# MCG-NJU/SparseBEV

Hardware: AMD Instinct MI355X
Metric: decoder samples/sec (6-cam T=8 900q r50_704x256, 6 layers, features resident in HBM) (higher is better)
Workload: dtype f32 (the two mixing GEMMs: f16x3 = fp32-class (default): fp32 operands as scaled fp16 hi + lo images, 3 products (hl, lh, hh), f32 accumulate on the 16-bit matrix core (csrc/gemm_bf16s.hip); max and rms error vs fp64 below the exact f32 MFMA kernels (tests/test_gpu_bf16s.py); mixing generator + out-; 1 GPU; c2: r50_704x256, 900 queries, T=8, bs=1 per GPU, 6 decoder layers, random-init weights, NCHW (reference layout, relayout inside the step: on demand -- only the feature units the sample points read) feature input; global_batch=1, parallelism=sample-sharded x1, launches_per_layer=6, query_order=False, shuffled_queries=False, relayout=on-demand

## Files before the change

### include/sbev_hip.h

```cpp
#ifndef SBEV_HIP_H
#define SBEV_HIP_H

#include <stdint.h>

#ifdef __cplusplus
extern "C" {
#endif

#define SBEV_ABI_VERSION 1
#define SBEV_MAX_LEVELS 5
#define SBEV_MAX_POINTS 32
#define SBEV_MAX_FRAMES 16

typedef void* sbev_stream_t;

enum sbev_status {
    SBEV_OK = 0,
    SBEV_EINVAL = -1,
    SBEV_ELAUNCH = -2,
    SBEV_ENODEV = -3,
    SBEV_EFAULT = -4
};

enum sbev_dtype { SBEV_F32 = 0, SBEV_BF16 = 1, SBEV_F16 = 2, SBEV_U8 = 3 };
// ... 372 lines not shown
typedef struct sbev_decoder_config {
    int32_t B, Q, T, N, G, P, L;
    int32_t D, H, ffn;
    int32_t num_classes, code_size, num_layers, out_points;
    int32_t attn_in_rows;
    int32_t feat_dtype;
    int32_t hw[SBEV_MAX_LEVELS][2];
    float image_h, image_w, eps_homo;
    int32_t gemm_mode;
    int32_t n_slots;
    int32_t frame_slots[SBEV_MAX_FRAMES];
    int32_t overlap;
    double pc_range[6];
    const int32_t* slot_table;
} sbev_decoder_config;

typedef struct sbev_decoder_weights {
    const float *pe0_w, *pe0_b, *pe1_g, *pe1_b, *pe3_w, *pe3_b, *pe4_g, *pe4_b;
    const float *attn_in_w, *attn_in_b;
    const float *attn_out_w, *attn_out_b;
    const float *samp_w, *samp_b;
    const float *pg_w, *pg_b, *op_w, *op_b;
    const uint16_t *pg_w2, *op_w2;
    const float *ffn0_w, *ffn0_b, *ffn1_w, *ffn1_b;
    const float *norm1_g, *norm1_b, *norm2_g, *norm2_b, *norm3_g, *norm3_b;
    const float *cls0_w, *cls0_b, *cls1_g, *cls1_b, *cls3_w, *cls3_b, *cls4_g, *cls4_b, *cls6_w, *cls6_b;
    const float *reg0_w, *reg0_b, *reg2_w, *reg2_b, *reg4_w, *reg4_b;
    const float *chain_pack;
    const uint16_t *pg_ws;
    const uint16_t *op_wp;
    const float *pg_wdown;
    const float *op_nscale;
    const float *pg_xscale;
} sbev_decoder_weights;

int64_t sbev_decoder_chain_pack_floats(const sbev_decoder_config* cfg);
int sbev_decoder_chain_pack(const sbev_decoder_config* cfg, const sbev_decoder_weights* weights, float* out, sbev_stream_t stream);
int sbev_decoder_row_chain(int enable);

int sbev_decoder_chain_pair(int enable);
int64_t sbev_decoder_chain_pair_timeouts(void);
int64_t sbev_decoder_chain_pair_faults(void);
int64_t sbev_decoder_chain_pair_faults_ack(void);
int sbev_decoder_out_fold(int enable);
int sbev_linear_out8_min_rows(int rows);
int sbev_debug_out_fold_drop(int enable);
int sbev_init(void);
int sbev_debug_chain_pair_drop(int enable);

int sbev_decoder_launches_per_layer(const sbev_decoder_config* cfg, const sbev_decoder_weights* weights);

int sbev_decoder_switches(int32_t* out, int capacity);

int sbev_decoder_mixed_up_log2(const sbev_decoder_config* cfg);

int64_t sbev_decoder_workspace_bytes(const sbev_decoder_config* cfg);

int sbev_decoder_forward(const sbev_decoder_config* cfg, const sbev_decoder_weights* weights,
                         const void* const* feats_nhwc, const float* query_bbox, const float* query_feat,
                         const float* time_diff, const float* lidar2img, const float* vel_div,
                         const uint8_t* attn_mask, float* cls_out, float* bbox_out,
                         void* workspace, int64_t workspace_bytes, sbev_stream_t stream);

typedef struct sbev_lazy_feats {
    const void* const* table;
    int32_t index[SBEV_MAX_LEVELS];
    const void* src[SBEV_MAX_LEVELS];
} sbev_lazy_feats;
int sbev_decoder_lazy_supported(const sbev_decoder_config* cfg);
int sbev_decoder_lazy_scan_launch(int enable);
int sbev_decoder_forward_lazy(const sbev_decoder_config* cfg, const sbev_decoder_weights* weights, void* const* feats_nhwc,
                              const sbev_lazy_feats* lazy, const float* query_bbox, const float* query_feat,
                              const float* time_diff, const float* lidar2img, const float* vel_div,
                              const uint8_t* attn_mask, float* cls_out, float* bbox_out,
                              void* workspace, int64_t workspace_bytes, sbev_stream_t stream);
int64_t sbev_prefix_cache_bytes(const sbev_decoder_config* cfg);
int sbev_decoder_forward_cached(const sbev_decoder_config* cfg, const sbev_decoder_weights* weights, void* const* feats_nhwc,
                                const sbev_lazy_feats* lazy, const float* query_bbox, const float* query_feat,
                                const float* time_diff, const float* lidar2img, const float* vel_div,
                                const uint8_t* attn_mask, float* cls_out, float* bbox_out,
                                void* workspace, int64_t workspace_bytes, sbev_stream_t stream, void* cache, int64_t cache_bytes);
int sbev_decoder_prefix_planned(const sbev_decoder_config* cfg, const sbev_decoder_weights* weights, int cache_given, int mask_given,
                                int lazy_given);
int64_t sbev_lazy_relayout_tiles(int n_levels, const int32_t* hw_pixels, int64_t n_images, int channels);
int sbev_sample_and_project_touch(const float* query_bbox, const float* offset, int64_t ld_offset,
                                  const float* scale_logits, int64_t ld_logits,
                                  const float* time_diff, const float* lidar2img, const double* pc_range,
                                  int B, int Q, int T, int N, int G, int P, int L,
                                  float image_h, float image_w, float eps,
                                  float* loc_bp, float* weights_bp, const int32_t* hw, uint32_t* need, sbev_stream_t stream);
int sbev_nchw_to_nhwc_lazy(const void* const* table, const int32_t* index, const void* const* src, void* const* out, int n_levels,
                           const int32_t* hw_pixels, int64_t n_images, int channels, int dtype, uint32_t* need, uint32_t* done, int first,
                           int last, sbev_stream_t stream);

typedef struct sbev_graph sbev_graph;
int sbev_decoder_capture(const sbev_decoder_config* cfg, const sbev_decoder_weights* weights,
                         const void* const* feats_nhwc, const float* query_bbox, const float* query_feat,
                         const float* time_diff, const float* lidar2img, const float* vel_div,
                         const uint8_t* attn_mask, float* cls_out, float* bbox_out,
                         void* workspace, int64_t workspace_bytes, sbev_stream_t stream, sbev_graph** out);
int sbev_capture_begin(sbev_stream_t stream);
int sbev_capture_end(sbev_stream_t stream, sbev_graph** out);
int sbev_graph_launch(sbev_graph* graph, sbev_stream_t stream);
int64_t sbev_graph_num_nodes(const sbev_graph* graph);
int sbev_graph_destroy(sbev_graph* graph);

int sbev_profile_sampler(int enable);
int sbev_profile_sampler_read(float* ms, int max_n);
int sbev_profile_stride(int every_n_calls);
int sbev_profile_read(int kind, float* ms, int max_n);

enum sbev_frames_layout { SBEV_FRAMES_NCHW = 0, SBEV_FRAMES_NHWC = 1 };
int sbev_pool_insert_frames(const void* const* table, const int32_t* index, const void* const* src, void* const* out, int n_frames,
                            int n_levels, const int32_t* hw_pixels, int B, int n_views, int channels, int src_layout, int src_dtype,
                            int dst_dtype, const int32_t* insert, int n_slots, sbev_stream_t stream);

int sbev_pool_insert(const void* const* table, const int32_t* index, const void* const* src, void* const* out, int n_levels,
                     const int32_t* hw_pixels, int B, int n_views, int channels, int dtype, const int32_t* insert, int n_slots,
                     sbev_stream_t stream);

#define SBEV_FRONT_ROW_BYTES 64
int sbev_image_front_plan(int n, int H, int W, int div, int64_t* out);
int sbev_image_front(const void* src, int src_dtype, void* dst, int dst_dtype, int n, int H, int W, int div, const float* mean,
                     const float* std, int to_rgb, int colour_on, const void* table, sbev_stream_t stream);

#ifdef __cplusplus
}
#endif
#endif
```

### sparsebev_amd/_lib.py

```python
import ctypes
import os

import torch

_HERE = os.path.dirname(os.path.abspath(__file__))
LIB_PATH = os.environ.get('SBEV_LIB_PATH') or os.path.join(_HERE, 'csrc', 'libsbev_hip.so')

_c_i64p = ctypes.POINTER(ctypes.c_int64)
_c_i32p = ctypes.POINTER(ctypes.c_int32)
_vp = ctypes.c_void_p

SIGNATURES = {
    'sbev_abi_version': (ctypes.c_int, []),
    'sbev_set_box_convention': (ctypes.c_int, [ctypes.c_int]),
    'sbev_get_box_convention': (ctypes.c_int, []),
    'sbev_last_error': (ctypes.c_char_p, []),
    'sbev_device_count': (ctypes.c_int, []),
    'sbev_msmv_fwd': (ctypes.c_int, [ctypes.POINTER(_vp), _c_i32p, ctypes.c_int, ctypes.c_int,
                                     ctypes.c_int64, ctypes.c_int, ctypes.c_int, ctypes.c_int, ctypes.c_int,
                                     ctypes.c_int, _c_i64p, ctypes.c_int64, _c_i64p, ctypes.c_int64,
                                     _vp, _vp, _vp, ctypes.c_int, ctypes.c_int, ctypes.c_int, _vp]),
    'sbev_project_select': (ctypes.c_int, [_vp, _vp, ctypes.c_int, ctypes.c_int, ctypes.c_int, ctypes.c_int,
                                           ctypes.c_int, ctypes.c_int, ctypes.c_float, ctypes.c_float, ctypes.c_float,
                                           _vp, _vp, _vp, _vp, _vp]),
    'sbev_sampling_front': (ctypes.c_int, [_vp, _vp, ctypes.c_int64, _vp, ctypes.c_int64, _vp, ctypes.POINTER(ctypes.c_double),
                                           ctypes.c_int, ctypes.c_int, ctypes.c_int, ctypes.c_int, ctypes.c_int, ctypes.c_int,
                                           _vp, _vp, _vp]),
    'sbev_linear_f32': (ctypes.c_int, [_vp, _vp, _vp, _vp, _vp, ctypes.c_int64, ctypes.c_int, ctypes.c_int,
                                       ctypes.c_int64, ctypes.c_int64, ctypes.c_int64, ctypes.c_int, _vp]),
    'sbev_linear_splitk_workspace': (ctypes.c_int64, [ctypes.c_int64, ctypes.c_int, ctypes.c_int]),
    'sbev_linear_splitk_f32': (ctypes.c_int, [_vp, _vp, _vp, _vp, _vp, _vp, ctypes.c_float, _vp,
                                              ctypes.c_int64, ctypes.c_int, ctypes.c_int, ctypes.c_int64, ctypes.c_int64,
                                              ctypes.c_int, ctypes.c_int, _vp, _vp]),
    'sbev_layer_norm_f32': (ctypes.c_int, [_vp, _vp, _vp, ctypes.c_float, _vp, _vp, ctypes.c_int64, ctypes.c_int,
                                           ctypes.c_int, _vp]),
    'sbev_ln_linear_f32': (ctypes.c_int, [_vp, _vp, _vp, ctypes.c_float, ctypes.c_int, _vp, _vp, _vp, _vp, _vp, _vp,
                                          ctypes.c_int64, ctypes.c_int, ctypes.c_int, ctypes.c_int64, ctypes.c_int64,
                                          ctypes.c_int, _vp]),
    'sbev_adaptive_mixing_f32': (ctypes.c_int, [_vp, _vp, _vp, ctypes.c_int64, ctypes.c_int, ctypes.c_int, ctypes.c_int,
                                                ctypes.c_int, ctypes.c_float, _vp]),
    'sbev_sasa_f32': (ctypes.c_int, [_vp, ctypes.c_int64, _vp, ctypes.POINTER(ctypes.c_double), _vp, _vp,
                                     ctypes.c_int, ctypes.c_int, ctypes.c_int, ctypes.c_int, _vp]),
    'sbev_refine_bbox': (ctypes.c_int, [_vp, _vp, _vp, _vp, ctypes.c_int, ctypes.c_int, ctypes.c_int, _vp]),
    'sbev_nchw_to_nhwc_f32': (ctypes.c_int, [_vp, _vp, ctypes.c_int64, ctypes.c_int, ctypes.c_int, _vp]),
    'sbev_nchw_to_nhwc_f32_indirect': (ctypes.c_int, [_vp, ctypes.c_int, _vp, ctypes.c_int64, ctypes.c_int, ctypes.c_int, _vp]),
    'sbev_nchw_to_nhwc_f32_multi_indirect': (ctypes.c_int, [_vp, ctypes.c_int, _c_i32p, ctypes.POINTER(_vp), ctypes.c_int64, ctypes.c_int, _c_i32p, _vp]),
    'sbev_nchw_to_nhwc_b16': (ctypes.c_int, [_vp, _vp, ctypes.c_int64, ctypes.c_int, ctypes.c_int, _vp]),
    'sbev_nchw_to_nhwc_b16_indirect': (ctypes.c_int, [_vp, ctypes.c_int, _vp, ctypes.c_int64, ctypes.c_int, ctypes.c_int, _vp]),
    'sbev_copy_indirect': (ctypes.c_int, [_vp, ctypes.c_int, _c_i32p, ctypes.POINTER(_vp), _c_i64p, _vp]),
    'sbev_finish_outputs': (ctypes.c_int, [_vp, _vp, _vp, _vp, ctypes.c_int64, ctypes.c_int64, _vp]),
    'sbev_finish_outputs_indirect': (ctypes.c_int, [_vp, ctypes.c_int, ctypes.c_int, _vp, _vp, ctypes.c_int64, ctypes.c_int64, _vp]),
    'sbev_linear3_ln_relu_f32': (ctypes.c_int, [_vp, ctypes.c_int64, _vp, _vp, _vp, _vp, ctypes.c_float, _vp,
                                                ctypes.c_int64, ctypes.c_int, _vp]),
    'sbev_decoder_workspace_bytes': (ctypes.c_int64, [_vp]),
    'sbev_decoder_launches_per_layer': (ctypes.c_int, [_vp, _vp]),
    'sbev_decoder_switches': (ctypes.c_int, [_c_i32p, ctypes.c_int]),
    'sbev_decoder_forward': (ctypes.c_int, [_vp, _vp, ctypes.POINTER(_vp), _vp, _vp, _vp, _vp, _vp, _vp, _vp, _vp,
                                            _vp, ctypes.c_int64, _vp]),
    'sbev_decoder_forward_lazy': (ctypes.c_int, [_vp, _vp, ctypes.POINTER(_vp), _vp, _vp, _vp, _vp, _vp, _vp, _vp, _vp, _vp,
                                                 _vp, ctypes.c_int64, _vp]),
    'sbev_decoder_forward_cached': (ctypes.c_int, [_vp, _vp, ctypes.POINTER(_vp), _vp, _vp, _vp, _vp, _vp, _vp, _vp, _vp, _vp,
                                                   _vp, ctypes.c_int64, _vp, _vp, ctypes.c_int64]),
    'sbev_prefix_cache_bytes': (ctypes.c_int64, [_vp]),
    'sbev_decoder_prefix_planned': (ctypes.c_int, [_vp, _vp, ctypes.c_int, ctypes.c_int, ctypes.c_int]),
    'sbev_decoder_lazy_supported': (ctypes.c_int, [_vp]),
    'sbev_decoder_lazy_scan_launch': (ctypes.c_int, [ctypes.c_int]),
    'sbev_lazy_relayout_tiles': (ctypes.c_int64, [ctypes.c_int, _c_i32p, ctypes.c_int64, ctypes.c_int]),
    'sbev_sample_and_project_touch': (ctypes.c_int, [_vp, _vp, ctypes.c_int64, _vp, ctypes.c_int64, _vp, _vp,
                                                     ctypes.POINTER(ctypes.c_double), ctypes.c_int, ctypes.c_int, ctypes.c_int,
                                                     ctypes.c_int, ctypes.c_int, ctypes.c_int, ctypes.c_int,
                                                     ctypes.c_float, ctypes.c_float, ctypes.c_float, _vp, _vp, _c_i32p, _vp, _vp]),
    'sbev_nchw_to_nhwc_lazy': (ctypes.c_int, [_vp, _c_i32p, ctypes.POINTER(_vp), ctypes.POINTER(_vp), ctypes.c_int, _c_i32p, ctypes.c_int64,
                                              ctypes.c_int, ctypes.c_int, _vp, _vp, ctypes.c_int, ctypes.c_int, _vp]),
    'sbev_init': (ctypes.c_int, []),
    'sbev_decoder_out_fold': (ctypes.c_int, [ctypes.c_int]),
    'sbev_linear_out8_min_rows': (ctypes.c_int, [ctypes.c_int]),
    'sbev_debug_out_fold_drop': (ctypes.c_int, [ctypes.c_int]),
    'sbev_profile_sampler': (ctypes.c_int, [ctypes.c_int]),
    'sbev_profile_stride': (ctypes.c_int, [ctypes.c_int]),
    'sbev_profile_sampler_read': (ctypes.c_int, [ctypes.POINTER(ctypes.c_float), ctypes.c_int]),
    'sbev_splitk_reduce_f32': (ctypes.c_int, [_vp, ctypes.c_int, _vp, _vp, _vp, _vp, ctypes.c_float, _vp, ctypes.c_int64,
                                              ctypes.c_int, ctypes.c_int, _vp]),
    'sbev_split_bf16x3_weights': (ctypes.c_int, [_vp, _vp, ctypes.c_int64, ctypes.c_int, _vp]),
    'sbev_linear_bf16x3_strip_ok': (ctypes.c_int, [ctypes.c_int64, ctypes.c_int, ctypes.c_int]),
    'sbev_linear_bf16x3_strip': (ctypes.c_int, [_vp, _vp, _vp, _vp, ctypes.c_int64, ctypes.c_int, ctypes.c_int, ctypes.c_int64,
                                                ctypes.c_int, _vp]),
    'sbev_linear_bf16x3': (ctypes.c_int, [_vp, _vp, _vp, _vp, _vp, ctypes.c_int64, ctypes.c_int, ctypes.c_int,
                                          ctypes.c_int64, ctypes.c_int64, ctypes.c_int, _vp]),
    'sbev_linear_splitk_bf16x3': (ctypes.c_int, [_vp, _vp, _vp, _vp, _vp, _vp, ctypes.c_float, _vp, ctypes.c_int64, ctypes.c_int,
                                                 ctypes.c_int, ctypes.c_int64, ctypes.c_int, ctypes.c_int, _vp, _vp]),
    'sbev_bf16s_image_elems': (ctypes.c_int64, [ctypes.c_int64, ctypes.c_int, ctypes.c_int]),
    'sbev_split_bf16s_rows': (ctypes.c_int, [_vp, ctypes.c_int64, _vp, ctypes.c_int64, ctypes.c_int, ctypes.c_int, _vp]),
    'sbev_pack_bf16s_frags': (ctypes.c_int, [_vp, ctypes.c_int64, _vp, ctypes.c_int, ctypes.c_int, ctypes.c_int, _vp]),
    'sbev_linear_gen_weight_stationary': (ctypes.c_int, [ctypes.c_int]),
    'sbev_linear_bf16s_gen_ok': (ctypes.c_int, [ctypes.c_int64, ctypes.c_int, ctypes.c_int]),
    'sbev_linear_bf16s_gen': (ctypes.c_int, [_vp, _vp, _vp, _vp, ctypes.c_int64, ctypes.c_int, ctypes.c_int, ctypes.c_int64,
                                             ctypes.c_int, ctypes.c_int, _vp]),
    'sbev_decoder_mixed_up_log2': (ctypes.c_int, [_vp]),
    'sbev_pack_f16s_frags': (ctypes.c_int, [_vp, ctypes.c_int64, _vp, _vp, ctypes.c_int, ctypes.c_int, ctypes.c_int, _vp]),
    'sbev_linear_f16s_gen': (ctypes.c_int, [_vp, _vp, _vp, _vp, _vp, _vp, ctypes.c_int64, ctypes.c_int, ctypes.c_int, ctypes.c_int64,
                                            ctypes.c_int, ctypes.c_int, _vp]),
    'sbev_f16s_pairs': (ctypes.c_int, [_vp, _vp, ctypes.c_int64, ctypes.c_int, _vp]),
    'sbev_f16s_tensor_scale': (ctypes.c_int, [_vp, ctypes.c_int64, ctypes.c_int64, ctypes.c_int, _vp, _vp]),
    'sbev_gemm_tn_f16s_ok': (ctypes.c_int, [ctypes.c_int64, ctypes.c_int64, ctypes.c_int64]),
    'sbev_gemm_tn_f16s': (ctypes.c_int, [_vp, ctypes.c_int64, _vp, _vp, ctypes.c_int64, _vp, _vp, ctypes.c_int64,
                                         ctypes.c_int64, ctypes.c_int64, ctypes.c_int64, ctypes.c_int, _vp]),
    'sbev_adaptive_mixing_bwd_max_f32': (ctypes.c_int, [_vp, _vp, _vp, _vp, _vp, _vp, ctypes.c_int64, ctypes.c_int, ctypes.c_int, ctypes.c_int,
                                                        ctypes.c_int, ctypes.c_float, _vp]),
    'sbev_adaptive_mixing_pairs_f16': (ctypes.c_int, [_vp, _vp, _vp, ctypes.c_int64, ctypes.c_int, ctypes.c_int, ctypes.c_int, ctypes.c_int,
                                                      ctypes.c_float, ctypes.c_int, _vp]),
    'sbev_linear_splitk_f16s': (ctypes.c_int, [_vp, ctypes.c_int, ctypes.c_int, _vp, _vp, _vp, _vp, _vp, _vp, ctypes.c_float, _vp, ctypes.c_int64, ctypes.c_int,
                                               ctypes.c_int, ctypes.c_int64, ctypes.c_int, ctypes.c_int, _vp, _vp]),
    'sbev_f16s_out_scale': (ctypes.c_int, [_vp, ctypes.c_int, _vp, ctypes.c_int, _vp]),
    'sbev_linear_splitk_f16s_xdev': (ctypes.c_int, [_vp, _vp, _vp, _vp, _vp, _vp, _vp, _vp, ctypes.c_float, _vp, ctypes.c_int64, ctypes.c_int,
                                                    ctypes.c_int, ctypes.c_int64, ctypes.c_int, ctypes.c_int, _vp, _vp]),
    'sbev_linear_bf16s_out_ok': (ctypes.c_int, [ctypes.c_int64, ctypes.c_int, ctypes.c_int]),
    'sbev_linear_bf16s_out_plan': (ctypes.c_int, [ctypes.c_int64, ctypes.c_int, ctypes.c_int]),
    'sbev_linear_gen_plan': (ctypes.c_int, [ctypes.c_int64, ctypes.c_int, ctypes.c_int, ctypes.c_int64, ctypes.c_int, ctypes.c_int, ctypes.c_int,
                                            _c_i32p, ctypes.c_int]),
    'sbev_linear_splitk_bf16s': (ctypes.c_int, [_vp, _vp, _vp, _vp, _vp, _vp, ctypes.c_float, _vp, ctypes.c_int64, ctypes.c_int,
                                                ctypes.c_int, ctypes.c_int64, ctypes.c_int, ctypes.c_int, _vp, _vp]),
    'sbev_msmv_bwd': (ctypes.c_int, [ctypes.POINTER(_vp), ctypes.POINTER(_vp), _c_i32p, ctypes.c_int,
                                     ctypes.c_int64, ctypes.c_int, ctypes.c_int, ctypes.c_int, ctypes.c_int,
                                     ctypes.c_int, _c_i64p, ctypes.c_int64, _c_i64p, ctypes.c_int64,
                                     _vp, _vp, _vp, _vp, _vp, _vp]),
    'sbev_msmv_fwd_ring': (ctypes.c_int, [ctypes.POINTER(_vp), _c_i32p, ctypes.c_int, ctypes.c_int,
                                          ctypes.c_int64, ctypes.c_int, ctypes.c_int, ctypes.c_int, ctypes.c_int,
                                          ctypes.c_int, _c_i64p, ctypes.c_int64, _c_i64p, ctypes.c_int64,
                                          _vp, _vp, _vp, ctypes.c_int, ctypes.c_int, ctypes.c_int, _c_i32p, ctypes.c_int, _vp]),
    'sbev_msmv_fwd_pool': (ctypes.c_int, [ctypes.POINTER(_vp), _c_i32p, ctypes.c_int, ctypes.c_int,
                                          ctypes.c_int64, ctypes.c_int, ctypes.c_int, ctypes.c_int, ctypes.c_int,
                                          ctypes.c_int, _c_i64p, ctypes.c_int64, _c_i64p, ctypes.c_int64,
                                          _vp, _vp, _vp, ctypes.c_int, ctypes.c_int, ctypes.c_int, _vp, ctypes.c_int, _vp]),
    'sbev_sample_mix_pool': (ctypes.c_int, [ctypes.POINTER(_vp), _c_i32p, ctypes.c_int, ctypes.c_int,
                                            ctypes.c_int64, ctypes.c_int, ctypes.c_int, ctypes.c_int, ctypes.c_int, ctypes.c_int, ctypes.c_int,
                                            _c_i64p, ctypes.c_int64, _c_i64p, ctypes.c_int64, _vp, _vp, _c_i32p, _vp, ctypes.c_int,
                                            _vp, _vp, ctypes.c_int, ctypes.c_float, ctypes.c_int, ctypes.c_int, _vp, _vp]),
    'sbev_sample_and_project': (ctypes.c_int, [_vp, _vp, ctypes.c_int64, _vp, ctypes.c_int64, _vp, _vp,
                                               ctypes.POINTER(ctypes.c_double), ctypes.c_int, ctypes.c_int, ctypes.c_int,
                                               ctypes.c_int, ctypes.c_int, ctypes.c_int, ctypes.c_int,
                                               ctypes.c_float, ctypes.c_float, ctypes.c_float, _vp, _vp, _vp]),
    'sbev_decoder_capture': (ctypes.c_int, [_vp, _vp, ctypes.POINTER(_vp), _vp, _vp, _vp, _vp, _vp, _vp, _vp, _vp, _vp, ctypes.c_int64, _vp, _vp]),
    'sbev_capture_begin': (ctypes.c_int, [_vp]),
    'sbev_capture_end': (ctypes.c_int, [_vp, _vp]),
    'sbev_graph_launch': (ctypes.c_int, [_vp, _vp]),
    'sbev_graph_num_nodes': (ctypes.c_int64, [_vp]),
    'sbev_graph_destroy': (ctypes.c_int, [_vp]),
# ... 167 lines not shown
```

### sparsebev_amd/csrc/decoder.hip

```cpp
#include <atomic>
#include <cmath>
#include <cstdlib>
#include <cstring>
#include "sbev_common.hpp"

#include <mutex>
#include <vector>

namespace {

struct Carver {
    char* base;
    size_t off = 0;
    explicit Carver(void* p) : base(static_cast<char*>(p)) {}
    float* take(size_t n_floats) {
        float* r = reinterpret_cast<float*>(base + off);
        off += (n_floats * sizeof(float) + 255) / 256 * 256;
        return r;
    }
};

struct Buffers {
    float *t0, *t1, *x, *x1, *x2, *x3, *qkvt, *att, *so, *wbp, *loc, *sampled, *params, *mixed, *slabs,
        *h, *c0, *c1, *r0, *r1, *reg, *bbox, *x1s, *xsc, *pair_x, *folded;
    uint32_t* pair_sync;
    int32_t* order;
    uint32_t *touch_need, *touch_done;
    size_t bytes;
};

bool lazy_plan_of(const sbev_decoder_config& c, sbev::LazyPlan* p) {
    if (c.n_slots > 0 || c.G != 4 || c.D != 256) return false;
    int32_t s[SBEV_MAX_LEVELS];
    for (int l = 0; l < c.L; ++l) s[l] = c.hw[l][0] * c.hw[l][1];
    return sbev::lazy_plan(c.L, s, (long long)c.B * c.T * c.N, c.D, p);
}

int out_proj_splits(long long M, int N, int K) { return sbev_linear_splitk_plan(M, N, K); }

Buffers carve(const sbev_decoder_config& c, void* ws) {
    Carver k(ws);
    const size_t BQ = (size_t)c.B * c.Q, D = c.D;
    const int Cg = c.D / c.G, Pin = c.T * c.P;
    const size_t pgN = (size_t)c.G * (Cg * Cg + Pin * c.out_points);
    const size_t mixN = (size_t)c.G * c.out_points * Cg;
    Buffers b{};
    b.t0 = k.take(BQ * D); b.t1 = k.take(BQ * D);
    b.x = k.take(BQ * D); b.x1 = k.take(BQ * D); b.x2 = k.take(BQ * D); b.x3 = k.take(BQ * D);
    b.qkvt = k.take(BQ * (size_t)c.attn_in_rows);
    b.att = k.take(BQ * D);
    b.so = k.take(BQ * (size_t)(c.G * c.P * (3 + c.L)));
    b.wbp = k.take(BQ * c.T * c.G * c.P * c.L);
    b.loc = k.take(BQ * c.T * c.G * c.P * 3);
    b.sampled = k.take(BQ * c.G * Pin * Cg);
    b.params = k.take(BQ * pgN);
    b.mixed = k.take(BQ * mixN);
    {
        int sl = out_proj_splits(BQ, c.D, (int)mixN);
        const int sl2 = sbev_linear_bf16s_out_plan((int64_t)BQ, c.D, (int)mixN);
        sl = sl2 > sl ? sl2 : sl;
        b.slabs = k.take((size_t)sl * BQ * D);
    }
    b.h = k.take(BQ * c.ffn);
    b.c0 = k.take(BQ * D); b.c1 = k.take(BQ * D); b.r0 = k.take(BQ * D); b.r1 = k.take(BQ * D);
    b.reg = k.take(BQ * c.code_size);
    b.bbox = k.take(BQ * 10);
    b.x1s = k.take(2 * BQ * D + 64 * (size_t)D);
    b.xsc = k.take(64);
    b.pair_x = k.take((size_t)sbev::chain_pair_floats((long long)BQ));
    b.pair_sync = reinterpret_cast<uint32_t*>(k.take((size_t)sbev::chain_pair_sync_words((long long)BQ)));
    b.order = reinterpret_cast<int32_t*>(k.take(BQ));
    b.folded = k.take(BQ * D);
    sbev::LazyPlan lp;
    if (lazy_plan_of(c, &lp)) {
        b.touch_need = reinterpret_cast<uint32_t*>(k.take(lp.base[lp.n_levels]));
        b.touch_done = reinterpret_cast<uint32_t*>(k.take(lp.base[lp.n_levels]));
    }
    b.bytes = k.off;
    return b;
}

struct Prefix {
    uint32_t* hdr;
    float *qb, *qf, *x0, *att0, *params0;
    size_t bytes;
};
Prefix carve_prefix(const sbev_decoder_config& c, void* cache) {
    Carver k(cache);
    const size_t BQ = (size_t)c.B * c.Q, D = c.D;
    const int Cg = c.D / c.G, Pin = c.T * c.P;
    Prefix f{};
    f.hdr = reinterpret_cast<uint32_t*>(k.take(sbev::PFX_DIRTY + sbev::PFX_NW));
    f.qb = k.take(BQ * 10);
    f.qf = k.take(BQ * D);
    f.x0 = k.take(BQ * D);
    f.att0 = k.take(BQ * D);
    f.params0 = k.take(BQ * (size_t)c.G * (Cg * Cg + Pin * c.out_points));
    f.bytes = k.off;
    return f;
}

struct WatchArgs {
    const uint32_t* q[2];
    uint32_t* copy[2];
    uint32_t words[2];
    uint32_t* hdr;
};
__global__ __launch_bounds__(256) void prefix_watch_kernel(const WatchArgs a) {
    const uint32_t armed = a.hdr[sbev::PFX_ARMED], force = a.hdr[sbev::PFX_FORCE];
    uint32_t differed = 0;
#pragma unroll
    for (int s = 0; s < 2; ++s) {
        const uint4* q = reinterpret_cast<const uint4*>(a.q[s]);
        uint4* cp = reinterpret_cast<uint4*>(a.copy[s]);
        const uint32_t n16 = a.words[s] / 4;
        for (uint32_t i = blockIdx.x * 256u + threadIdx.x; i < n16; i += sbev::PFX_NW * 256u) {
            const uint4 v = q[i], o = cp[i];
            if (((v.x ^ o.x) | (v.y ^ o.y)) | ((v.z ^ o.z) | (v.w ^ o.w))) {
                cp[i] = v;
                differed = 1;
            }
        }
        const uint32_t t = 4 * n16 + threadIdx.x;
        if (blockIdx.x == 0 && t < a.words[s] && a.q[s][t] != a.copy[s][t]) {
            a.copy[s][t] = a.q[s][t];
            differed = 1;
        }
    }
    const int any = __syncthreads_or((int)differed);
    if (threadIdx.x == 0) {
        a.hdr[sbev::PFX_DIRTY + blockIdx.x] = (any != 0 || armed == 0 || force != 0) ? 1u : 0u;
        if (blockIdx.x == 0) a.hdr[sbev::PFX_ARMED] = 1u;
    }
}

std::atomic<int> g_fuse_sample_mix{1};
std::atomic<int> g_fuse_l5_f32{getenv("SBEV_NO_FUSE_L5F32") ? 0 : 1};

std::atomic<int> g_query_order{getenv("SBEV_QUERY_ORDER") ? (atoi(getenv("SBEV_QUERY_ORDER")) == 2 ? 2 : atoi(getenv("SBEV_QUERY_ORDER")) != 0) : 0};

std::atomic<int> g_row_chain{1};
std::atomic<int> g_lazy_scan_launch{getenv("SBEV_LAZY_SCAN_LAUNCH") ? 1 : 0};

int validate(const sbev_decoder_config* c) {
    SBEV_REQUIRE(c != nullptr, "sbev_decoder: null config");
    SBEV_REQUIRE(c->B >= 1 && c->Q >= 1 && c->T >= 1 && c->N >= 1 && c->G >= 1 && c->P >= 1, "sbev_decoder: bad sizes");
    SBEV_REQUIRE(c->L >= 1 && c->L <= SBEV_MAX_LEVELS, "sbev_decoder: num_levels %d", c->L);
    SBEV_REQUIRE(c->D % (4 * c->G) == 0 && c->D % c->H == 0 && c->D / c->H == 32, "sbev_decoder: embed_dims %d / heads %d (head_dim must be 32)", c->D, c->H);
    SBEV_REQUIRE(c->D / c->G == 64 && c->out_points == 128, "sbev_decoder: built for 64 channels per group and 128 out points");
    SBEV_REQUIRE(c->attn_in_rows >= 3 * c->D + c->H && c->attn_in_rows % 4 == 0, "sbev_decoder: attn_in_rows %d", c->attn_in_rows);
    SBEV_REQUIRE(c->code_size == 10, "sbev_decoder: code_size %d (the box kernels are built for the 10-wide box code)", c->code_size);
    SBEV_REQUIRE(c->num_layers >= 1 && c->num_classes >= 1 && c->ffn % 4 == 0, "sbev_decoder: head sizes");
    SBEV_REQUIRE(c->gemm_mode >= SBEV_GEMM_F32 && c->gemm_mode <= SBEV_GEMM_F16X4, "sbev_decoder: gemm_mode %d", c->gemm_mode);
    SBEV_REQUIRE(!c->slot_table || (c->n_slots > 0 && c->T <= SBEV_MAX_FRAMES), "sbev_decoder: slot_table (keyed frame pool) needs n_slots > 0 and T <= %d",
                 SBEV_MAX_FRAMES);
    return SBEV_OK;
}

struct Aux {
    hipStream_t stream = nullptr;
    hipEvent_t ev[8] = {};
    bool ok = false;
};
Aux& aux() {
    static Aux a;
    static std::once_flag once;
    std::call_once(once, [] {
        bool ok = hipStreamCreateWithFlags(&a.stream, hipStreamNonBlocking) == hipSuccess;
        for (auto& e : a.ev) ok = ok && hipEventCreateWithFlags(&e, hipEventDisableTiming) == hipSuccess;
        a.ok = ok;
    });
    return a;
}
inline int hip_ok(hipError_t e, const char* what) {
    if (e == hipSuccess) return SBEV_OK;
    sbev::set_error("%s: %s", what, hipGetErrorString(e));
    return SBEV_ELAUNCH;
}

struct ConfigPyramid {
    int64_t sbo[SBEV_MAX_LEVELS], sv[SBEV_MAX_LEVELS];
    sbev::PyramidDesc d;
    ConfigPyramid(const sbev_decoder_config& c, const void* const* feats, const float* loc, const float* weights)
        : d{feats, &c.hw[0][0], c.L, c.feat_dtype, c.N, c.D / c.G, c.Q, c.P, c.G, sbo, c.D / c.G, sv, c.D, loc, weights,
            c.n_slots > 0 && !c.slot_table ? c.frame_slots : nullptr, c.n_slots, c.slot_table} {
        for (int l = 0; l < c.L; ++l) {
            sv[l] = (int64_t)c.hw[l][0] * c.hw[l][1] * c.D;
            sbo[l] = sv[l] * c.N;
        }
    }
    ConfigPyramid(const ConfigPyramid&) = delete;
};

#define TRY(expr)                 \
    do {                          \
        int st__ = (expr);        \
        if (st__ != SBEV_OK) return st__; \
    } while (0)

}

static bool launch_profiling_on();

namespace sbev {
struct ProfCallScope {
    bool prev;
    ProfCallScope();
    ~ProfCallScope();
};
// ... 22 lines not shown
    return s;
}

extern "C" int sbev_decoder_switches(int32_t* out, int capacity) {
    constexpr int n = (int)(sizeof(sbev::Switches) / sizeof(int32_t));
    static_assert(sizeof(sbev::Switches) == n * sizeof(int32_t), "sbev::Switches: int32_t fields only");
    const sbev::Switches s = read_switches();
    if (out && capacity > 0) std::memcpy(out, &s, sizeof(int32_t) * (capacity < n ? capacity : n));
    return n;
}

struct StepPlan {
    int nimg;
    int64_t BQ;
    int pgN, mixN, soN;
    int splits;
    bool fork, fork_pg;
    bool chain;
    bool fused;
    int order_mode;
    bool pg_strip;
    bool pack_launch;
    bool gen_ws;
    bool scan_in_gen;
    bool fold_wanted;
    bool grouped;
    bool prefix;
    int out8_min_rows;
    int launches_per_layer;
};

static StepPlan plan_step(const sbev_decoder_config& c, const sbev_decoder_weights& w, bool lazy, bool aux_ok, const sbev::Switches& sw,
                          bool cache_usable = false) {
    StepPlan p{};
    p.nimg = c.gemm_mode == SBEV_GEMM_BF16X6 ? 3 : c.gemm_mode == SBEV_GEMM_BF16X3S ? 2 : c.gemm_mode == SBEV_GEMM_F16X3 ? 4
             : c.gemm_mode == SBEV_GEMM_F16X4 ? 5 : 0;
    const int D = c.D, Cg = c.D / c.G, Pin = c.T * c.P;
    p.BQ = (int64_t)c.B * c.Q;
    p.pgN = c.G * (Cg * Cg + Pin * c.out_points);
    p.mixN = c.G * c.out_points * Cg;
    p.soN = c.G * c.P * (3 + c.L);
    p.splits = out_proj_splits(p.BQ, D, p.mixN);
    p.fork = c.overlap != 0 && aux_ok;
    p.fork_pg = c.overlap == 1 && aux_ok;
    p.chain = sw.row_chain != 0 && w.chain_pack != nullptr && !p.fork && sbev::row_chain_supported(c) && sbev::row_chain_pays(p.BQ);
    p.fused = sw.fuse_sample_mix != 0 && sample_mix_fusable(c, sw.fuse_l5_f32 != 0);
    p.order_mode = p.chain && p.fused && c.Q <= sbev_query_order_max() ? sw.query_order : 0;
    p.pg_strip = c.gemm_mode == SBEV_GEMM_BF16X3 && sbev_linear_bf16x3_strip_ok(p.BQ, p.pgN, D) != 0;
    p.pack_launch = p.nimg ? !(p.nimg >= 4 && p.chain) : p.pg_strip;
    p.gen_ws = p.nimg != 0 && sw.gen_weight_stationary != 0 && sbev::gen_ws_shape_ok(p.BQ, D, p.pgN, p.nimg);
    p.scan_in_gen = lazy && p.chain && p.nimg >= 4 && sw.lazy_scan_launch == 0 && p.BQ <= 1024 && p.gen_ws;
    p.fold_wanted = p.chain && p.nimg >= 4 && sw.chain_pair != 0 && sw.out_fold != 0;
    p.grouped = !p.fork && (D == 256 || D == 512) && ((p.BQ + 127) / 128) * ((D + 127) / 128) < 256;
    p.out8_min_rows = sw.out8_min_rows;
    p.prefix = cache_usable && p.chain && p.gen_ws;
    p.launches_per_layer = (p.chain ? 6 : 17) + (p.fused ? 0 : 1) + (p.pack_launch ? 1 : 0) + (p.order_mode == 1 ? 1 : 0);
    return p;
}

extern "C" int sbev_decoder_launches_per_layer(const sbev_decoder_config* cfg, const sbev_decoder_weights* w) {
    if (validate(cfg) != SBEV_OK || !w) return -1;
    return plan_step(*cfg, *w, false, true, read_switches()).launches_per_layer;
}

extern "C" int sbev_decoder_mixed_up_log2(const sbev_decoder_config* cfg) {
    if (!cfg || cfg->G < 1 || cfg->out_points < 1 || cfg->D < cfg->G) return 0;
    const double bound = std::sqrt((double)cfg->out_points * (cfg->D / cfg->G));
    int e = 0;
    while (std::ldexp(bound, e + 1) < 65504.0 && e < 15) ++e;
    return e;
}

extern "C" int64_t sbev_prefix_cache_bytes(const sbev_decoder_config* cfg) {
    if (validate(cfg) != SBEV_OK) return -1;
    return (int64_t)carve_prefix(*cfg, nullptr).bytes;
}

extern "C" int sbev_decoder_prefix_planned(const sbev_decoder_config* cfg, const sbev_decoder_weights* w, int cache_given, int mask_given,
                                           int lazy_given) {
    if (validate(cfg) != SBEV_OK || !w) return -1;
    return plan_step(*cfg, *w, lazy_given != 0, true, read_switches(), cache_given && !mask_given && !launch_profiling_on()).prefix ? 1 : 0;
}

extern "C" int64_t sbev_decoder_workspace_bytes(const sbev_decoder_config* cfg) {
    if (validate(cfg) != SBEV_OK) return -1;
    sbev::chain_pair_prepare();
    return (int64_t)carve(*cfg, nullptr).bytes;
}

namespace {

struct Step {
    const sbev_decoder_config& c;
    const sbev_decoder_weights& w;
    const StepPlan& p;
    const Buffers& b;
    const void* const* feats_nhwc;
    const float *query_bbox, *query_feat, *time_diff, *lidar2img, *vel_div;
    const uint8_t* attn_mask;
    float *cls_out, *bbox_out;
    const sbev_lazy_feats* lazy;
    const Prefix* pf;
    sbev_stream_t stream;
    Aux& ax;
    hipStream_t s_main = reinterpret_cast<hipStream_t>(stream);
    sbev_stream_t s_aux = p.fork ? reinterpret_cast<sbev_stream_t>(ax.stream) : stream;
    int evi = 0;
    sbev::LazyPlan lplan{};
    const ConfigPyramid pyramid{c, feats_nhwc, b.loc, b.wbp};
    const int mixed_up = sbev_decoder_mixed_up_log2(&c), D = c.D, Cg = c.D / c.G, Pin = c.T * c.P;
    const float eps = 1e-5f;
    const float* bbox = query_bbox;
    const float* feat = query_feat;
    bool pe0_done = false;
    hipEvent_t ev_cls = nullptr;
    float* params = b.params;
    const uint32_t* skip = nullptr;

    float* cls_of(int layer) const { return cls_out + (int64_t)layer * p.BQ * c.num_classes; }
    float* box_of(int layer) const { return bbox_out + (int64_t)layer * p.BQ * c.code_size; }
    int feat_esize() const { return c.feat_dtype == SBEV_F32 ? 4 : 2; }

    int fork_to_aux() {
        hipEvent_t e = ax.ev[(evi++) & 7];
        TRY(hip_ok(hipEventRecord(e, s_main), "hipEventRecord"));
        return hip_ok(hipStreamWaitEvent(ax.stream, e, 0), "hipStreamWaitEvent");
    }
    int record_on_aux(hipEvent_t* ev) {
        *ev = ax.ev[(evi++) & 7];
        return hip_ok(hipEventRecord(*ev, ax.stream), "hipEventRecord");
    }
    int join(hipEvent_t ev) { return ev ? hip_ok(hipStreamWaitEvent(s_main, ev, 0), "hipStreamWaitEvent") : SBEV_OK; }
    sbev::LazyScan lazy_scan(int layer) const {
        if (!lazy) return {};
        return {&lplan, lazy->table, lazy->index, lazy->src, const_cast<void* const*>(feats_nhwc), feat_esize(), b.touch_need, b.touch_done,
                layer + 1 == c.num_layers};
    }
    int lazy_move(const sbev::LazyScan& scan, bool first) { return scan.plan ? sbev::launch_lazy_relayout(scan, first, s_main) : SBEV_OK; }

    int generator_bf16x3(sbev_stream_t st) {
        if (!p.pg_strip) return sbev_linear_bf16x3(b.x1, w.pg_w2, w.pg_b, nullptr, params, p.BQ, p.pgN, D, D, p.pgN, 0, st);
        uint16_t* x2 = reinterpret_cast<uint16_t*>(b.x1s);
        TRY(sbev_split_bf16x3_weights(b.x1, x2, p.BQ, D, st));
        return sbev_linear_bf16x3_strip(x2, w.pg_w2, w.pg_b, params, p.BQ, p.pgN, D, p.pgN, 0, st);
    }
    int generator_bf16s(sbev_stream_t st, const sbev::LazyScan* scan) {
        uint16_t* xs = reinterpret_cast<uint16_t*>(b.x1s);
        if (p.pack_launch) {
            TRY(p.nimg >= 4 ? sbev_pack_f16s_frags(b.x1, D, xs, const_cast<float*>(w.pg_xscale), (int)p.BQ, D, 2, st)
                            : sbev_pack_bf16s_frags(b.x1, D, xs, (int)p.BQ, D, p.nimg, st));
        }
        return sbev::launch_gen_gemm({{xs, w.pg_xscale}, {w.pg_ws, w.pg_wdown}, w.pg_b, params, p.BQ, p.pgN, D, p.pgN, 0, p.nimg, p.gen_ws, scan, skip},
                                     reinterpret_cast<hipStream_t>(st));
    }
    int generator(sbev_stream_t st, const sbev::LazyScan* scan) {
        if (p.nimg) return generator_bf16s(st, scan);
        if (c.gemm_mode == SBEV_GEMM_BF16X3) return generator_bf16x3(st);
        return sbev_linear_f32(b.x1, w.pg_w, w.pg_b, nullptr, params, p.BQ, p.pgN, D, D, D, p.pgN, 0, st);
    }

    int gather(sbev_stream_t st) {
        return sbev::msmv_fwd(pyramid.d, (int64_t)c.B * c.T * c.G, b.sampled, SBEV_OUT_MIX, c.T, c.G, st);
    }
    int gather_and_mix(sbev_stream_t st, const int32_t* order, hipEvent_t params_ready = nullptr) {
        if (!p.fused) TRY(gather(st));
        TRY(join(params_ready));
        if (!p.fused && p.nimg >= 4) return sbev_adaptive_mixing_pairs_f16(b.sampled, params, b.mixed, p.BQ, c.G, Pin, Cg, c.out_points, eps, mixed_up, st);
        if (!p.fused) return sbev_adaptive_mixing_f32(b.sampled, params, b.mixed, p.BQ, c.G, Pin, Cg, c.out_points, eps, st);
        return sbev::sample_mix(pyramid.d, c.B, c.T, c.G, params, b.mixed, c.out_points, eps, p.nimg >= 4 ? ldexpf(1.f, mixed_up) : 0.f, order, st);
    }

    int out_projection_slabs(sbev::OutProjResult* r) {
        *r = {0, false};
        if (p.nimg) {
            const bool f16 = p.nimg >= 4;
            const bool fold = p.fold_wanted && sbev::out_fold_shape_ok(p.BQ, p.mixN) && sbev::chain_fault_word_ready();
            const sbev::OutProj o{{f16 ? sbev::SplitImageX::F16_PAIRS : sbev::SplitImageX::F32_HOST_EXP, b.mixed, p.mixN, f16 ? mixed_up : 0, nullptr},
                                  w.op_wp, f16 ? w.op_nscale : nullptr, p.BQ, p.mixN, p.nimg, b.slabs, p.out8_min_rows,
                                  fold ? b.pair_sync + sbev::chain_fold_sync_offset(p.BQ) : nullptr, fold ? b.folded : nullptr};
            return sbev::launch_out_proj_slabs(o, r, s_main);
        }
        if (c.gemm_mode == SBEV_GEMM_BF16X3)
            return sbev::launch_splitk_slabs_bf16x3(b.mixed, w.op_w2, p.BQ, D, p.mixN, p.mixN, p.splits, b.slabs, &r->used, s_main);
        return sbev::launch_splitk_slabs(b.mixed, w.op_w, p.BQ, D, p.mixN, p.mixN, p.mixN, p.splits, b.slabs, &r->used, s_main);
    }
    int out_projection(sbev_stream_t st) {
        if (p.nimg >= 4)
            return sbev_linear_splitk_f16s(b.mixed, 1, mixed_up, w.op_wp, w.op_nscale, w.op_b, b.x1, w.norm2_g, w.norm2_b, eps, b.x2, p.BQ, D, p.mixN,
                                           p.mixN, 0, p.nimg - 1, b.slabs, st);
        if (p.nimg)
            return sbev_linear_splitk_bf16s(b.mixed, w.op_wp, w.op_b, b.x1, w.norm2_g, w.norm2_b, eps, b.x2, p.BQ, D, p.mixN, p.mixN,
                                            0, p.nimg, b.slabs, st);
        if (c.gemm_mode == SBEV_GEMM_BF16X3)
            return sbev_linear_splitk_bf16x3(b.mixed, w.op_w2, w.op_b, b.x1, w.norm2_g, w.norm2_b, eps, b.x2, p.BQ, D, p.mixN, p.mixN,
                                             0, p.splits, b.slabs, st);
        return sbev_linear_splitk_f32(b.mixed, w.op_w, w.op_b, b.x1, w.norm2_g, w.norm2_b, eps, b.x2, p.BQ, D, p.mixN, p.mixN, p.mixN,
                                      0, p.splits, b.slabs, st);
    }

    int layer_chain(int layer) {
        if (p.order_mode != 0 && (layer == 0 || p.order_mode == 1)) TRY(sbev_query_order(bbox, c.code_size, c.pc_range, c.B, c.Q, b.order, stream));
        const bool cached = pf && layer == 0;
        float* att = cached ? pf->att0 : b.att;
        params = cached ? pf->params0 : b.params;
        skip = cached ? pf->hdr : nullptr;
        TRY(sbev::launch_sasa(b.qkvt, c.attn_in_rows, bbox, c.pc_range, attn_mask, att, c.B, c.Q, c.H, D / c.H, skip, s_main));
        TRY(sbev::launch_chain_attn(c, w, att, cached ? pf->x0 : b.x, b.x1, bbox, time_diff, lidar2img, b.loc, b.wbp, eps, s_main,
                                    p.nimg >= 4 ? reinterpret_cast<uint16_t*>(b.x1s) : nullptr, p.nimg >= 4 ? w.pg_xscale : nullptr, b.pair_sync,
                                    lazy ? &lplan : nullptr, lazy ? b.touch_need : nullptr));
        const bool ride = p.scan_in_gen && layer > 0;
        SBEV_REQUIRE(!(ride && skip), "sbev_decoder_forward: a generator that carries a relayout scan cannot skip");
        const sbev::LazyScan scan = lazy_scan(layer);
        if (!ride) TRY(lazy_move(scan, layer == 0));
        TRY(generator(stream, ride ? &scan : nullptr));
        TRY(gather_and_mix(stream, p.order_mode != 0 ? b.order : nullptr));
        sbev::OutProjResult op;
        TRY(out_projection_slabs(&op));
        TRY(sbev::launch_chain_tail(c, w, op.folded ? b.folded : b.slabs, op.used, b.x1, bbox, c.T > 1 ? vel_div : nullptr, b.x3, cls_of(layer), box_of(layer),
                                    layer + 1 < c.num_layers, b.x, b.qkvt, eps, s_main, b.pair_x, b.pair_sync));
        bbox = box_of(layer);
        return SBEV_OK;
    }

    int layer_ops(int layer) {
        if (!pe0_done) TRY(sbev_linear3_ln_relu_f32(bbox, layer == 0 ? 10 : c.code_size, w.pe0_w, w.pe0_b, w.pe1_g, w.pe1_b, eps, b.t0, p.BQ, D, stream));
        pe0_done = false;
        TRY(sbev_linear_f32(b.t0, w.pe3_w, w.pe3_b, nullptr, b.t1, p.BQ, D, D, D, D, D, 0, stream));
        TRY(sbev_ln_linear_f32(b.t1, w.pe4_g, w.pe4_b, eps, 1, feat, b.x, w.attn_in_w, w.attn_in_b, nullptr, b.qkvt,
                               p.BQ, c.attn_in_rows, D, D, c.attn_in_rows, 0, stream));
        TRY(sbev_sasa_f32(b.qkvt, c.attn_in_rows, bbox, c.pc_range, attn_mask, b.att, c.B, c.Q, c.H, D / c.H, stream));
        TRY(sbev_linear_f32(b.att, w.attn_out_w, w.attn_out_b, b.x, b.t1, p.BQ, D, D, D, D, D, 0, stream));
        TRY(sbev_ln_linear_f32(b.t1, w.norm1_g, w.norm1_b, eps, 0, nullptr, b.x1, w.samp_w, w.samp_b, nullptr, b.so,
                               p.BQ, p.soN, D, D, p.soN, 0, stream));
        hipEvent_t ev_pg = nullptr;
        if (p.fork_pg) TRY(fork_to_aux());
        TRY(generator(p.fork_pg ? s_aux : stream, nullptr));
        if (p.fork_pg) TRY(record_on_aux(&ev_pg));
        TRY(sbev::launch_sample_and_project(bbox, b.so, p.soN, b.so + c.G * c.P * 3, p.soN, time_diff, lidar2img, c.pc_range,
                                            c.B, c.Q, c.T, c.N, c.G, c.P, c.L, c.image_h, c.image_w, c.eps_homo, b.loc, b.wbp,
                                            lazy ? &lplan : nullptr, lazy ? b.touch_need : nullptr, c.hw, s_main));
        TRY(lazy_move(lazy_scan(layer), layer == 0));
        TRY(gather_and_mix(stream, nullptr, ev_pg));
        TRY(out_projection(stream));
        TRY(join(ev_cls));
        TRY(sbev_linear_f32(b.x2, w.ffn0_w, w.ffn0_b, nullptr, b.h, p.BQ, c.ffn, D, D, D, c.ffn, 1, stream));
        TRY(sbev_linear_f32(b.h, w.ffn1_w, w.ffn1_b, b.x2, b.t1, p.BQ, D, c.ffn, c.ffn, c.ffn, D, 0, stream));
        TRY(p.grouped ? branches_grouped(layer) : branches_forked(layer));
        bbox = box_of(layer);
        feat = b.x3;
        return SBEV_OK;
    }

    sbev_linear_problem problem(const float* X, const float* W, const float* bias, float* Y, int N, int relu) const {
        return sbev_linear_problem{X, W, bias, nullptr, Y, p.BQ, N, D, D, D, N, relu};
    }
    int branches_grouped(int layer) {
        const bool ln_fused = sbev::ln_linear_fusable(p.BQ, D, D);
        if (!ln_fused) TRY(sbev_layer_norm_f32(b.t1, w.norm3_g, w.norm3_b, eps, nullptr, b.x3, p.BQ, D, 0, stream));
        const float* x = ln_fused ? b.t1 : b.x3;
        const sbev_linear_problem g1[2] = {problem(x, w.cls0_w, w.cls0_b, b.c0, D, 0), problem(x, w.reg0_w, w.reg0_b, b.r0, D, 1)};
        const sbev::LnPrologue norm3{w.norm3_g, w.norm3_b, eps, 0, nullptr, b.x3};
        TRY(ln_fused ? sbev::launch_linear_group(g1, 2, &norm3, s_main) : sbev_linear_group_f32(g1, 2, stream));
        TRY(sbev::launch_ln_and_linear(b.c0, w.cls1_g, w.cls1_b, eps, 1, b.c1, p.BQ, D, b.r0, w.reg2_w, w.reg2_b, b.r1, D, D, 1, s_main));
        const sbev_linear_problem g2[2] = {problem(b.c1, w.cls3_w, w.cls3_b, b.c0, D, 0), problem(b.r1, w.reg4_w, w.reg4_b, b.reg, c.code_size, 0)};
        TRY(sbev_linear_group_f32(g2, 2, stream));
        TRY(sbev::launch_ln_and_refine(b.c0, w.cls4_g, w.cls4_b, eps, 1, b.c1, p.BQ, D,
                                       bbox, b.reg, c.T > 1 ? vel_div : nullptr, box_of(layer), c.Q, c.code_size, s_main));
        if (layer + 1 == c.num_layers)
            return sbev_linear_f32(b.c1, w.cls6_w, w.cls6_b, nullptr, cls_of(layer), p.BQ, c.num_classes, D, D, D, c.num_classes, 0, stream);
        TRY(sbev::launch_linear_and_lin3(b.c1, w.cls6_w, w.cls6_b, cls_of(layer), p.BQ, c.num_classes, D, 0,
                                         box_of(layer), c.code_size, w.pe0_w, w.pe0_b, w.pe1_g, w.pe1_b, eps, b.t0, D, s_main));
        pe0_done = true;
        return SBEV_OK;
    }
    int branches_forked(int layer) {
        TRY(sbev_ln_linear_f32(b.t1, w.norm3_g, w.norm3_b, eps, 0, nullptr, b.x3, w.cls0_w, w.cls0_b, nullptr, b.c0,
                               p.BQ, D, D, D, D, 0, stream));
        if (p.fork) TRY(fork_to_aux());
        TRY(sbev_layer_norm_f32(b.c0, w.cls1_g, w.cls1_b, eps, nullptr, b.c1, p.BQ, D, 1, s_aux));
        TRY(sbev_linear_f32(b.c1, w.cls3_w, w.cls3_b, nullptr, b.c0, p.BQ, D, D, D, D, D, 0, s_aux));
        TRY(sbev_layer_norm_f32(b.c0, w.cls4_g, w.cls4_b, eps, nullptr, b.c1, p.BQ, D, 1, s_aux));
        TRY(sbev_linear_f32(b.c1, w.cls6_w, w.cls6_b, nullptr, cls_of(layer), p.BQ, c.num_classes, D, D, D, c.num_classes, 0, s_aux));
        if (p.fork) TRY(record_on_aux(&ev_cls));
        TRY(sbev_linear_f32(b.x3, w.reg0_w, w.reg0_b, nullptr, b.r0, p.BQ, D, D, D, D, D, 1, stream));
        TRY(sbev_linear_f32(b.r0, w.reg2_w, w.reg2_b, nullptr, b.r1, p.BQ, D, D, D, D, D, 1, stream));
        TRY(sbev_linear_f32(b.r1, w.reg4_w, w.reg4_b, nullptr, b.reg, p.BQ, c.code_size, D, D, D, c.code_size, 0, stream));
        return sbev_refine_bbox(bbox, b.reg, c.T > 1 ? vel_div : nullptr, box_of(layer), c.B, c.Q, c.code_size, stream);
    }

    int prefix_watch() {
        const WatchArgs a{{reinterpret_cast<const uint32_t*>(query_bbox), reinterpret_cast<const uint32_t*>(query_feat)},
                          {reinterpret_cast<uint32_t*>(pf->qb), reinterpret_cast<uint32_t*>(pf->qf)},
                          {(uint32_t)(p.BQ * 10), (uint32_t)(p.BQ * D)}, pf->hdr};
        hipLaunchKernelGGL(prefix_watch_kernel, dim3(sbev::PFX_NW), dim3(256), 0, s_main, a);
        return sbev::check_launch("prefix cache (watch)");
    }

    int run() {
        if (pf) TRY(prefix_watch());
        if (p.chain) TRY(sbev::launch_chain_front(c, w, query_bbox, query_feat, pf ? pf->x0 : b.x, b.qkvt, eps, s_main, pf ? pf->hdr : nullptr));
        for (int layer = 0; layer < c.num_layers; ++layer) TRY(p.chain ? layer_chain(layer) : layer_ops(layer));
        return join(ev_cls);
    }
};

}

static int decoder_forward_impl(const sbev_decoder_config* cfg, const sbev_decoder_weights* w,
                                const void* const* feats_nhwc, const float* query_bbox, const float* query_feat,
                                const float* time_diff, const float* lidar2img, const float* vel_div,
                                const uint8_t* attn_mask, float* cls_out, float* bbox_out,
                                void* workspace, int64_t workspace_bytes, sbev_stream_t stream, const sbev_lazy_feats* lazy,
                                void* cache = nullptr, int64_t cache_bytes = 0) {
    TRY(validate(cfg));
    const sbev_decoder_config& c = *cfg;
    SBEV_REQUIRE(w && feats_nhwc && query_bbox && query_feat && time_diff && lidar2img && cls_out && bbox_out && workspace,
                 "sbev_decoder_forward: null pointer");
    if (const unsigned faults = sbev::chain_pair_faults_pending()) {
        sbev_decoder_chain_pair(0);
        sbev::set_error("sbev_decoder_forward: %u pair-mode hand-off(s) of an EARLIER decoder step timed out -- that step's outputs are invalid; "
                        "pair mode is now off: acknowledge with sbev_decoder_chain_pair_faults_ack() and repeat the step", faults);
        return SBEV_EFAULT;
    }
    const sbev::ProfCallScope prof_scope;
    Aux& ax = aux();
    const bool cache_usable = cache && !attn_mask && !launch_profiling_on() && ((((uintptr_t)query_bbox) | ((uintptr_t)query_feat)) & 15) == 0;
    const StepPlan p = plan_step(c, *w, lazy != nullptr, ax.ok, read_switches(), cache_usable);
    SBEV_REQUIRE((((uintptr_t)workspace) & 255) == 0, "sbev_decoder_forward: workspace must be 256-byte aligned");
    SBEV_REQUIRE(cfg->gemm_mode != SBEV_GEMM_BF16X3 || (w->pg_w2 && w->op_w2), "sbev_decoder_forward: gemm_mode bf16x3 needs pg_w2 / op_w2");
    SBEV_REQUIRE(p.nimg == 0 || (w->pg_ws && w->op_wp), "sbev_decoder_forward: gemm_mode %d needs pg_ws / op_wp", cfg->gemm_mode);
    SBEV_REQUIRE(p.nimg < 4 || (w->pg_wdown && w->op_nscale && w->pg_xscale), "sbev_decoder_forward: gemm_mode %d needs pg_wdown / op_nscale / pg_xscale", cfg->gemm_mode);
    const Buffers b = carve(c, workspace);
    SBEV_REQUIRE((int64_t)b.bytes <= workspace_bytes, "sbev_decoder_forward: workspace too small (%lld < %zu)", (long long)workspace_bytes, b.bytes);

    Prefix pf{};
    if (p.prefix) {
        pf = carve_prefix(c, cache);
        SBEV_REQUIRE((((uintptr_t)cache) & 255) == 0, "sbev_decoder_forward_cached: cache must be 256-byte aligned");
        SBEV_REQUIRE((int64_t)pf.bytes <= cache_bytes, "sbev_decoder_forward_cached: cache too small (%lld < %zu)", (long long)cache_bytes, pf.bytes);
        SBEV_REQUIRE(p.BQ * (int64_t)c.D < 0x7fffffffLL, "sbev_decoder_forward_cached: too many query words");
    }
    Step step{c, *w, p, b, feats_nhwc, query_bbox, query_feat, time_diff, lidar2img, vel_div, attn_mask, cls_out, bbox_out, lazy,
              p.prefix ? &pf : nullptr, stream, ax};
    if (lazy) {
        SBEV_REQUIRE(lazy_plan_of(c, &step.lplan) && b.touch_need, "sbev_decoder_forward_lazy: config not covered (dense pyramid, 4 groups of 64 channels)");
        for (int l = 0; l < c.L; ++l)
            SBEV_REQUIRE(feats_nhwc[l] && (((uintptr_t)feats_nhwc[l]) & 15) == 0 &&
                         (lazy->table ? lazy->index[l] >= 0 : (lazy->src[l] && (((uintptr_t)lazy->src[l]) & 15) == 0 && lazy->src[l] != feats_nhwc[l])),
                         "sbev_decoder_forward_lazy: level %d (16-byte aligned NCHW source and NHWC destination)", l);
        SBEV_REQUIRE(!lazy->table || (((uintptr_t)lazy->table) & 7) == 0, "sbev_decoder_forward_lazy: unaligned pointer table");
    }
    SBEV_REQUIRE(p.nimg == 0 || (sbev_linear_bf16s_gen_ok(p.BQ, p.pgN, c.D) && sbev_linear_bf16s_out_ok(p.BQ, c.D, p.mixN)),
                 "sbev_decoder_forward: gemm_mode %d does not cover this shape (rows %lld, generator %d x %d, out-projection %d x %d)",
                 cfg->gemm_mode, (long long)p.BQ, p.pgN, c.D, c.D, p.mixN);
    return step.run();
}

extern "C" int sbev_decoder_forward(const sbev_decoder_config* cfg, const sbev_decoder_weights* w,
                                    const void* const* feats_nhwc, const float* query_bbox, const float* query_feat,
                                    const float* time_diff, const float* lidar2img, const float* vel_div,
                                    const uint8_t* attn_mask, float* cls_out, float* bbox_out,
                                    void* workspace, int64_t workspace_bytes, sbev_stream_t stream) {
    return decoder_forward_impl(cfg, w, feats_nhwc, query_bbox, query_feat, time_diff, lidar2img, vel_div, attn_mask, cls_out, bbox_out, workspace,
                                workspace_bytes, stream, nullptr);
}

extern "C" int sbev_decoder_forward_lazy(const sbev_decoder_config* cfg, const sbev_decoder_weights* w, void* const* feats_nhwc,
                                         const sbev_lazy_feats* lazy, const float* query_bbox, const float* query_feat,
                                         const float* time_diff, const float* lidar2img, const float* vel_div,
                                         const uint8_t* attn_mask, float* cls_out, float* bbox_out,
                                         void* workspace, int64_t workspace_bytes, sbev_stream_t stream) {
    SBEV_REQUIRE(lazy, "sbev_decoder_forward_lazy: null source descriptor");
    return decoder_forward_impl(cfg, w, const_cast<const void* const*>(feats_nhwc), query_bbox, query_feat, time_diff, lidar2img, vel_div, attn_mask,
                                cls_out, bbox_out, workspace, workspace_bytes, stream, lazy);
}

extern "C" int sbev_decoder_forward_cached(const sbev_decoder_config* cfg, const sbev_decoder_weights* w, void* const* feats_nhwc,
                                           const sbev_lazy_feats* lazy, const float* query_bbox, const float* query_feat,
                                           const float* time_diff, const float* lidar2img, const float* vel_div,
                                           const uint8_t* attn_mask, float* cls_out, float* bbox_out,
                                           void* workspace, int64_t workspace_bytes, sbev_stream_t stream, void* cache, int64_t cache_bytes) {
    return decoder_forward_impl(cfg, w, const_cast<const void* const*>(feats_nhwc), query_bbox, query_feat, time_diff, lidar2img, vel_div, attn_mask,
                                cls_out, bbox_out, workspace, workspace_bytes, stream, lazy, cache, cache_bytes);
}

extern "C" int sbev_decoder_lazy_supported(const sbev_decoder_config* cfg) {
    sbev::LazyPlan p;
    return cfg && validate(cfg) == SBEV_OK && lazy_plan_of(*cfg, &p) ? 1 : 0;
}

namespace sbev {
static std::mutex g_prof_mu;
static int g_prof_mask = 0;
static int g_prof_stride = 1;
static long long g_prof_calls = 0;
static thread_local bool tl_prof_skip = false;
struct ProfEvent { hipEvent_t e0, e1; int kind; };
static std::vector<ProfEvent> g_prof_events;

bool profile_begin(hipStream_t s, hipEvent_t* e0, hipEvent_t* e1, int kind) {
    std::lock_guard<std::mutex> lk(g_prof_mu);
    if (!((g_prof_mask >> kind) & 1) || tl_prof_skip) return false;
    if (hipEventCreate(e0) != hipSuccess || hipEventCreate(e1) != hipSuccess) return false;
    (void)hipEventRecord(*e0, s);
    return true;
}
void profile_end(hipStream_t s, hipEvent_t e0, hipEvent_t e1, int kind) {
    (void)hipEventRecord(e1, s);
    std::lock_guard<std::mutex> lk(g_prof_mu);
    g_prof_events.push_back({e0, e1, kind});
}
}

static bool launch_profiling_on() {
    std::lock_guard<std::mutex> lk(sbev::g_prof_mu);
    return sbev::g_prof_mask != 0;
}

namespace sbev {
ProfCallScope::ProfCallScope() : prev(tl_prof_skip) {
    std::lock_guard<std::mutex> lk(g_prof_mu);
    if (g_prof_mask != 0 && g_prof_stride > 1) tl_prof_skip = (g_prof_calls++ % g_prof_stride) != 0;
}
ProfCallScope::~ProfCallScope() { tl_prof_skip = prev; }
}

extern "C" int sbev_profile_stride(int every_n_calls) {
    SBEV_REQUIRE(every_n_calls >= 1, "sbev_profile_stride: need n >= 1 (got %d)", every_n_calls);
    std::lock_guard<std::mutex> lk(sbev::g_prof_mu);
    sbev::g_prof_stride = every_n_calls;
    sbev::g_prof_calls = 0;
    return SBEV_OK;
}

extern "C" int sbev_decoder_lazy_scan_launch(int enable) { return g_lazy_scan_launch.exchange(enable ? 1 : 0, std::memory_order_relaxed); }

extern "C" int sbev_decoder_row_chain(int enable) {
    g_row_chain.store(enable != 0, std::memory_order_relaxed);
    return SBEV_OK;
}

extern "C" int sbev_decoder_fuse_sample_mix(int enable) {
    g_fuse_sample_mix.store(enable ? 1 : 0, std::memory_order_relaxed);
    return SBEV_OK;
}

extern "C" int sbev_decoder_query_order(int enable) {
    return g_query_order.exchange(enable == 2 ? 2 : enable ? 1 : 0, std::memory_order_relaxed);
}

extern "C" int sbev_profile_sampler(int enable) {
    std::lock_guard<std::mutex> lk(sbev::g_prof_mu);
    sbev::g_prof_mask = enable;
    return SBEV_OK;
}

extern "C" int sbev_profile_read(int kind, float* ms, int max_n) {
    std::lock_guard<std::mutex> lk(sbev::g_prof_mu);
    int n = 0;
    std::vector<sbev::ProfEvent> keep;
    for (auto& ev : sbev::g_prof_events) {
        if (ev.kind != kind) {
            keep.push_back(ev);
            continue;
        }
        float t = 0.f;
// ... 106 lines not shown
```

### sparsebev_amd/csrc/row_chain.hip

```cpp
#include "sbev_common.hpp"
#include "sample_point.hpp"
#include <mutex>
#include <atomic>
#include <cstdlib>

namespace {

constexpr int NWAVE = 8;
constexpr int DM = 256, FF = 512;
constexpr int LDX = DM + 8;
constexpr int LDH = FF + 8;
static_assert(2 * LDX >= LDH, "branch rows alias the ffn hidden rows");

constexpr int PV_OP_B = 0, PV_N2G = 256, PV_N2B = 512, PV_FFN0_B = 768, PV_FFN1_B = 1280, PV_N3G = 1536, PV_N3B = 1792,
              PV_CLS0_B = 2048, PV_CLS1G = 2304, PV_CLS1B = 2560, PV_CLS3_B = 2816, PV_CLS4G = 3072, PV_CLS4B = 3328,
              PV_CLS6_B = 3584, PV_REG0_B = 3648, PV_REG2_B = 3904, PV_REG4_B = 4160, PV_TAIL_END = 4224;
constexpr int PV_PE0_W = PV_TAIL_END, PV_PE0_B = PV_PE0_W + 768, PV_PE1G = PV_PE0_B + 256, PV_PE1B = PV_PE1G + 256,
              PV_PE3_B = PV_PE1B + 256, PV_PE4G = PV_PE3_B + 256, PV_PE4B = PV_PE4G + 256, PV_QKV_B = PV_PE4B + 256, PV_QKV_PAD = 832,
              PV_FRONT_END = PV_QKV_B + PV_QKV_PAD;
constexpr int PV_AOUT_B = 0, PV_N1G = 256, PV_N1B = 512, PV_SAMP_B = 768, PV_ATTN_END = 1024;
constexpr int PV_IMAGE_FLOATS = PV_FRONT_END + PV_ATTN_END;

enum Epi { EPI_FFN0, EPI_FFN1, EPI_BR1, EPI_BR2, EPI_OUT, EPI_PE3, EPI_QKV, EPI_AOUT, EPI_SAMP };
enum Pre { PRE_SLABS, PRE_FRONT, PRE_ATT };

struct Lin {
    const float* wp;
    int in_off, ld;
    int KH;
    int items;
    int chunks;
    int kh0, KHT;
};
struct Unit {
    Lin a, b;
    int epi;
    int col0;
};

#ifdef SBEV_CHAIN_TRACE
#define SBEV_TRACE(i) if ((blockIdx.x == 7 || blockIdx.x == 15) && lane == 0) a.trace[(blockIdx.x == 15 ? 64 * 512 : 0) + wave * 64 + (i)] = (long long)__builtin_amdgcn_s_memrealtime();
#else
#define SBEV_TRACE(i)
#endif

struct ChainArgs {
#ifdef SBEV_CHAIN_TRACE
    long long* trace;
#endif
    Unit units[8];
    Unit units_b[8];
    int n_units, pre, front;
    int n_pairs;
    float* pair_x;
    unsigned* pair_sync;
    unsigned* zero_words; int n_zero;
    int debug_drop;
    const float* warm;
    int warm_lines;
    const float* vec;
    int vec_off, vec_n;
    long long M;
    int Q;
    const float* slabs; int splits;
    const float* x1;
    float* x3;
    const float* bbox;
    const float* vel_div;
    float* cls_out;
    float* box_out;
    int num_classes;
    const float* feat;
    float* x;
    float* qkvt; int attn_in_rows;
    const float* att;
    float* x1_out;
    unsigned short* x1_frag;
    const float* x1_scale;
    float* so; int soN;
    sbev_ops::SamplePointArgs proj;
    float eps;
    uint32_t* skip_hdr;
};

constexpr int RING_SLOTS = 3;
constexpr int CHUNK_FLOATS = 1024;

template <int RG>
struct Lay {
    static constexpr int R = 4 * RG;
    static constexpr bool WIDE = RG > 1;
    static constexpr int MAX_SLOTS = WIDE ? 12 : 16;
    static constexpr int OFF_X2 = 0;
    static constexpr int OFF_X3 = OFF_X2 + R * LDX;
    static constexpr int OFF_H = OFF_X3 + R * LDX;
    static constexpr int OFF_C = OFF_H;
    static constexpr int OFF_R = OFF_H + R * LDX;
    static constexpr int OFF_P = OFF_H + 2 * R * LDX;
    static constexpr int LDS_FLOATS = OFF_P + MAX_SLOTS * R * 64;
    static constexpr int OFF_RING = LDS_FLOATS;
    static constexpr int OFF_DUMP = OFF_RING + (WIDE ? 0 : NWAVE * RING_SLOTS * CHUNK_FLOATS);
    static constexpr int OFF_PARAM = OFF_DUMP + NWAVE * 64;
    static constexpr int LDS_TOTAL_FLOATS = OFF_PARAM + PV_FRONT_END;
    static constexpr int RPW = (R + NWAVE - 1) / NWAVE;
    static_assert(LDS_TOTAL_FLOATS * 4 <= 160 * 1024, "LDS budget of one CU");
};
struct Offs { int x2, x3, h, c, r; };
template <int RG> constexpr Offs offs_of() { return Offs{Lay<RG>::OFF_X2, Lay<RG>::OFF_X3, Lay<RG>::OFF_H, Lay<RG>::OFF_C, Lay<RG>::OFF_R}; }

template <int RG>
__device__ __forceinline__ void warm_l2(const ChainArgs& a, int wave, int lane) {
    const int per_xcd = ((int)gridDim.x + 7) / 8;
    const int parts = per_xcd < 32 ? per_xcd : 32;
    const int part = ((int)blockIdx.x / 8) % parts;
    const int n = (a.warm_lines + parts - 1) / parts;
    const int l0 = part * n;
    const int l1 = min(a.warm_lines, l0 + n);
    const unsigned dump = (unsigned)(Lay<RG>::OFF_DUMP + wave * 64) * 4u;
    for (int l = l0 + wave * 64; l < l1; l += NWAVE * 64) {
        const int line = min(l + lane, l1 - 1);
        const unsigned voff = (unsigned)line * 128u;
        asm volatile(
            "s_mov_b32 m0, %0\n\t"
            "s_nop 0\n\t"
            "global_load_lds_dword %1, %2\n\t"
            :
            : "s"(dump), "v"(voff), "s"(a.warm)
            : "memory");
    }
}

struct Walk {
    int u, it, step;
};

__device__ __forceinline__ int unit_items(const Unit* U, int u) { return U[u].a.items + U[u].b.items; }

__device__ __forceinline__ void walk_settle(const ChainArgs& a, const Unit* U, Walk& w, int wave) {
    while (w.u < a.n_units && w.it >= unit_items(U, w.u)) {
        ++w.u;
        w.it = wave;
    }
}

__device__ __forceinline__ const float* item_weights(const Unit& un, int it) {
    const bool second = it >= un.a.items;
    const Lin& l = second ? un.b : un.a;
    const int j = it - (second ? un.a.items : 0);
    const int piece = l.KHT == l.KH ? j : (j / l.KH) * l.KHT + l.kh0 + j % l.KH;
    return l.wp + (long long)piece * (l.chunks * CHUNK_FLOATS);
}

__device__ __forceinline__ void issue_chunk(const float* g, unsigned lds_byte, unsigned voff) {
    asm volatile(
        "s_mov_b32 m0, %0\n\t"
        "s_nop 0\n\t"
        "global_load_lds_dwordx4 %1, %2\n\t"
        "global_load_lds_dwordx4 %1, %2 offset:1024\n\t"
        "global_load_lds_dwordx4 %1, %2 offset:2048\n\t"
        "global_load_lds_dwordx4 %1, %2 offset:3072\n\t"
        :
        : "s"(lds_byte), "v"(voff), "s"(g)
        : "memory");
}

struct Stream {
// ... 146 lines not shown
#pragma unroll
        for (int kh = 0; kh < KH; ++kh) t[c][kh] = P[(base + (cg0 + c) * KH + kh) * (R * 64) + row * 64 + lane];
#pragma unroll
    for (int c = 0; c < 4; ++c) {
        float s = 0.f;
#pragma unroll
        for (int kh = 0; kh < KH; ++kh) s += t[c][kh];
        v[c] = s + bias[bias0 + lane + 64 * c];
    }
}
template <int R>
__device__ __forceinline__ void gather4(float (&v)[4], const float* P, int base, int KH, int cg0, int row, int lane, const float* bias,
                                        int bias0) {
    if (KH == 1) gather4_t<1, R>(v, P, base, cg0, row, lane, bias, bias0);
    else if (KH == 2) gather4_t<2, R>(v, P, base, cg0, row, lane, bias, bias0);
    else gather4_t<4, R>(v, P, base, cg0, row, lane, bias, bias0);
}

template <int R>
__device__ __forceinline__ void gather4_raw(float (&v)[4], const float* P, int KH, int row, int lane) {
#pragma unroll
    for (int c = 0; c < 4; ++c) {
        float s = 0.f;
        for (int kh = 0; kh < KH; ++kh) s += P[(c * KH + kh) * (R * 64) + row * 64 + lane];
        v[c] = s;
    }
}

__device__ unsigned g_chain_pair_timeouts;
__device__ unsigned* g_chain_pair_fault_host;
constexpr unsigned PAIR_POLL_LIMIT = 1u << 20;

__device__ __forceinline__ void pair_store4(float* p, const float (&v)[4]) {
    const f32x4 q = {v[0], v[1], v[2], v[3]};
    asm volatile("global_store_dwordx4 %0, %1, off sc0 sc1\n\ts_nop 1" ::"v"(p), "v"(q) : "memory");
}
__device__ __forceinline__ void pair_load4(const float* p, float (&v)[4]) {
    f32x4 q;
    asm volatile("global_load_dwordx4 %0, %1, off sc0 sc1\n\ts_waitcnt vmcnt(0)" : "=v"(q) : "v"(p) : "memory");
    v[0] = q.x; v[1] = q.y; v[2] = q.z; v[3] = q.w;
}
__device__ __forceinline__ void pair_arrive(unsigned* word) {
    asm volatile("s_waitcnt vmcnt(0)" ::: "memory");
    __syncthreads();
    if (threadIdx.x == 0) __hip_atomic_fetch_add(word, 1u, __ATOMIC_RELAXED, __HIP_MEMORY_SCOPE_AGENT);
}
__device__ __forceinline__ void pair_wait(unsigned* word, unsigned arrivals) {
    if (threadIdx.x == 0) {
        unsigned n = 0;
        while (__hip_atomic_load(word, __ATOMIC_RELAXED, __HIP_MEMORY_SCOPE_AGENT) < arrivals) {
            __builtin_amdgcn_s_sleep(2);
            if (++n > PAIR_POLL_LIMIT) {
                __hip_atomic_fetch_add(&g_chain_pair_timeouts, 1u, __ATOMIC_RELAXED, __HIP_MEMORY_SCOPE_AGENT);
                unsigned* const host_word = g_chain_pair_fault_host;
                if (host_word) __hip_atomic_fetch_add(host_word, 1u, __ATOMIC_RELAXED, __HIP_MEMORY_SCOPE_SYSTEM);
                break;
            }
        }
    }
    __syncthreads();
}

__device__ __forceinline__ void store_rows(float* smem, int off, int ld, int row, int lane, const float (&v)[4]) {
#pragma unroll
    for (int c = 0; c < 4; ++c) smem[off + row * ld + lane + 64 * c] = v[c];
}

template <int RG>
__device__ __forceinline__ void pe0_row(const ChainArgs& a, float* smem, int row, int lane, float x0, float x1, float x2) {
    constexpr int OFF_PARAM = Lay<RG>::OFF_PARAM, OFF_C = Lay<RG>::OFF_C;
    const float* pv = smem + OFF_PARAM;
    const LnW lw(pv + PV_PE1G, pv + PV_PE1B, lane);
    float v[4];
#pragma unroll
    for (int c = 0; c < 4; ++c) {
        const int n = lane + 64 * c;
        const float* w = pv + PV_PE0_W + n * 3;
        v[c] = ((x0 * w[0] + x1 * w[1]) + x2 * w[2]) + pv[PV_PE0_B + n];
    }
    ln4(v, lw, a.eps, true);
    store_rows(smem, OFF_C, LDX, row, lane, v);
}

template <int PRE, int RG, bool PAIR = false>
__global__ __launch_bounds__(64 * NWAVE) void row_chain_kernel(const ChainArgs a) {
    using L = Lay<RG>;
    static_assert(!PAIR || (PRE == PRE_SLABS && RG > 1), "pair mode: the tail, wide row blocks");
    constexpr int R = L::R, RPW = L::RPW, OFF_X2 = L::OFF_X2, OFF_X3 = L::OFF_X3, OFF_H = L::OFF_H, OFF_C = L::OFF_C, OFF_R = L::OFF_R,
                  OFF_P = L::OFF_P, OFF_PARAM = L::OFF_PARAM;
    extern __shared__ __attribute__((aligned(16))) float smem[];
    const int lane = threadIdx.x & 63;
    const int wave = __builtin_amdgcn_readfirstlane(threadIdx.x >> 6);
    int pair = (int)blockIdx.x, member = 0;
    if constexpr (PAIR) {
        const int li = (int)blockIdx.x >> 3;
        pair = (li >> 1) * 8 + ((int)blockIdx.x & 7);
        member = li & 1;
        if (pair >= a.n_pairs) return;
        if (a.debug_drop && pair == 0 && member == 1) return;
    }
    const Unit* const U = (PAIR && member) ? a.units_b : a.units;
    unsigned* const pword = PAIR ? a.pair_sync + pair : nullptr;
    float* const px = PAIR ? a.pair_x + (long long)pair * (3 * R * DM) : nullptr;
    const long long row0 = (long long)pair * R;
    float* P = smem + OFF_P;
    if constexpr (PRE == PRE_FRONT) {
        if (a.skip_hdr) {
            const bool clean = sbev::prefix_clean(a.skip_hdr);
            if (blockIdx.x == 0 && threadIdx.x == 0) {
                uint32_t* n = a.skip_hdr + (clean ? sbev::PFX_HITS : sbev::PFX_MISSES);
                *n = *n + 1u;
            }
            if (clean) return;
        }
    }
    if (PRE == PRE_ATT && a.zero_words && blockIdx.x == 0)
        for (int i = threadIdx.x; i < a.n_zero; i += 64 * NWAVE) a.zero_words[i] = 0u;

    SBEV_TRACE(0)
    warm_l2<RG>(a, wave, lane);
    Stream st;
    st.U = U;
    st.iw = Walk{0, wave, 0};
    st.issued = st.used = st.islot = st.uslot = 0;
    st.ring_byte = (unsigned)(L::OFF_RING + wave * (RING_SLOTS * CHUNK_FLOATS)) * 4u;
    st.voff = (unsigned)lane * 16u;
    st.g = a.warm;
    st.nchunk = 8;
    stream_seek(a, st, wave);
    RChunk rb[RDEPTH];
    if constexpr (L::WIDE) {
#pragma unroll
        for (int d = 0; d < RDEPTH; ++d) {
#pragma unroll
            for (int m = 0; m < 4; ++m) rb[d].q[m] = make_float4(0.f, 0.f, 0.f, 0.f);
            stream_load(a, st, wave, lane, rb[d]);
        }
    } else {
        stream_issue(a, st, wave);
        stream_issue(a, st, wave);
        stream_issue(a, st, wave);
    }

    const float* pv = smem + OFF_PARAM;
    constexpr int PASSES = (PV_FRONT_END / 4 + 64 * NWAVE - 1) / (64 * NWAVE);
    float4 pq[PASSES];
#pragma unroll
    for (int j = 0; j < PASSES; ++j) {
        const int i4 = (int)threadIdx.x + j * 64 * NWAVE;
        pq[j] = *reinterpret_cast<const float4*>(a.vec + 4 * min(i4, a.vec_n / 4 - 1));
    }
    float4 t[RPW], r4[RPW];
    float v0[RPW][4], v1[RPW][4];
    float bx[RPW], by[RPW], bz[RPW];
    bool plive[RPW];
#pragma unroll
    for (int pi = 0; pi < RPW; ++pi) {
        const int prow = wave + pi * NWAVE;
        const long long pg = row0 + prow;
        plive[pi] = prow < R && pg < a.M;
        t[pi] = make_float4(0.f, 0.f, 0.f, 0.f); r4[pi] = t[pi];
#pragma unroll
        for (int c = 0; c < 4; ++c) v0[pi][c] = v1[pi][c] = 0.f;
        bx[pi] = by[pi] = bz[pi] = 0.f;
        if (PRE == PRE_SLABS) {
            if (plive[pi]) r4[pi] = *reinterpret_cast<const float4*>(a.x1 + pg * DM + lane * 4);
        } else if (plive[pi]) {
            const float* src = PRE == PRE_FRONT ? a.feat : a.att;
#pragma unroll
            for (int c = 0; c < 4; ++c) v0[pi][c] = src[pg * DM + lane + 64 * c];
            if (PRE == PRE_FRONT) { bx[pi] = a.bbox[pg * 10]; by[pi] = a.bbox[pg * 10 + 1]; bz[pi] = a.bbox[pg * 10 + 2]; }
            if (PRE == PRE_ATT) {
#pragma unroll
                for (int c = 0; c < 4; ++c) v1[pi][c] = a.x[pg * DM + lane + 64 * c];
            }
        }
    }
    if (PRE == PRE_SLABS) {
        constexpr int NB = 32 / RPW;
        for (int z0 = 0; z0 < a.splits; z0 += NB) {
            float4 q[RPW][NB];
#pragma unroll
            for (int pi = 0; pi < RPW; ++pi) {
                const long long pg = min(row0 + wave + pi * NWAVE, a.M - 1);
#pragma unroll
                for (int j = 0; j < NB; ++j)
                    q[pi][j] = *reinterpret_cast<const float4*>(a.slabs + ((long long)min(z0 + j, a.splits - 1) * a.M + pg) * DM + lane * 4);
            }
#pragma unroll
            for (int pi = 0; pi < RPW; ++pi)
#pragma unroll
                for (int j = 0; j < NB; ++j) asm volatile("" ::"v"(q[pi][j].x), "v"(q[pi][j].y), "v"(q[pi][j].z), "v"(q[pi][j].w));
#pragma unroll
            for (int pi = 0; pi < RPW; ++pi)
#pragma unroll
                for (int j = 0; j < NB; ++j) {
                    const float m = (z0 + j < a.splits && plive[pi]) ? 1.f : 0.f;
                    t[pi].x += q[pi][j].x * m; t[pi].y += q[pi][j].y * m; t[pi].z += q[pi][j].z * m; t[pi].w += q[pi][j].w * m;
                }
        }
// ... 32 lines not shown

    SBEV_TRACE(1)
    for (int u = 0; u < a.n_units; ++u) {
        const Unit& un = U[u];
        const int items = un.a.items + un.b.items;
        for (int it = wave; it < items; it += NWAVE) {
            const bool second = it >= un.a.items;
            if constexpr (L::WIDE) mma_item_wide<RG>(a, st, rb, second ? un.b : un.a, it - (second ? un.a.items : 0), smem, it, lane, wave);
            else mma_item(a, st, second ? un.b : un.a, it - (second ? un.a.items : 0), smem, it, lane, wave);
        }
        SBEV_TRACE(2 + 4 * u)
        __syncthreads();
        SBEV_TRACE(3 + 4 * u)
        if constexpr (PAIR) {
            if (un.epi == EPI_FFN1) {
                for (int row = wave; row < R; row += NWAVE) {
                    float v[4];
                    gather4_raw<R>(v, P, un.a.KH, row, lane);
                    pair_store4(px + (member * R + row) * DM + lane * 4, v);
                }
                pair_arrive(pword);
                pair_wait(pword, 2u);
            } else if (un.epi == EPI_PE3 && member == 0) {
                pair_wait(pword, 3u);
            }
        }
        for (int task = wave; task < 2 * R; task += NWAVE) {
            const int row = task % R, side = task / R;
            const long long g = row0 + row;
            const bool live = g < a.M;
            float v[4];
            if (PAIR && side != member && (un.epi == EPI_FFN0 || un.epi == EPI_BR1 || un.epi == EPI_BR2 || un.epi == EPI_OUT)) continue;
            switch (un.epi) {
            case EPI_FFN0: {
                gather4<R>(v, P, 0, un.a.KH, PAIR ? 0 : side * 4, row, lane, pv + PV_FFN0_B, side * 256);
#pragma unroll
                for (int c = 0; c < 4; ++c) smem[OFF_H + row * LDH + side * 256 + lane + 64 * c] = fmaxf(v[c], 0.f);
            } break;
            case EPI_FFN1: {
                if (side) break;
                const LnW lw(pv + PV_N3G, pv + PV_N3B, lane);
                float res[4];
#pragma unroll
                for (int c = 0; c < 4; ++c) res[c] = smem[OFF_X2 + row * LDX + lane + 64 * c];
                if constexpr (PAIR) {
                    float own[4], oth[4];
                    gather4_raw<R>(own, P, un.a.KH, row, lane);
                    pair_load4(px + ((1 - member) * R + row) * DM + lane * 4, oth);
#pragma unroll
                    for (int c = 0; c < 4; ++c) v[c] = ((member ? oth[c] : own[c]) + (member ? own[c] : oth[c])) + pv[PV_FFN1_B + lane + 64 * c];
                } else {
                    gather4<R>(v, P, 0, un.a.KH, 0, row, lane, pv + PV_FFN1_B, 0);
                }
#pragma unroll
                for (int c = 0; c < 4; ++c) v[c] += res[c];
                ln4(v, lw, a.eps, false);
                store_rows(smem, OFF_X3, LDX, row, lane, v);
                if (live && member == 0) {
#pragma unroll
                    for (int c = 0; c < 4; ++c) a.x3[g * DM + lane + 64 * c] = v[c];
                }
            } break;
            case EPI_BR1:
            case EPI_BR2: {
                const bool first = un.epi == EPI_BR1;
                if (side == 0) {
                    const LnW lw(pv + (first ? PV_CLS1G : PV_CLS4G), pv + (first ? PV_CLS1B : PV_CLS4B), lane);
                    gather4<R>(v, P, 0, un.a.KH, 0, row, lane, pv + (first ? PV_CLS0_B : PV_CLS3_B), 0);
                    ln4(v, lw, a.eps, true);
                    store_rows(smem, OFF_C, LDX, row, lane, v);
                } else {
                    gather4<R>(v, P, un.a.items, un.b.KH, 0, row, lane, pv + (first ? PV_REG0_B : PV_REG2_B), 0);
#pragma unroll
                    for (int c = 0; c < 4; ++c) v[c] = fmaxf(v[c], 0.f);
                    store_rows(smem, OFF_R, LDX, row, lane, v);
                }
            } break;
            case EPI_OUT: {
                if (side == 0) {
                    if (lane < a.num_classes) {
                        float s = 0.f;
                        for (int kh = 0; kh < un.a.KH; ++kh) s += P[kh * (R * 64) + row * 64 + lane];
                        if (live) a.cls_out[g * a.num_classes + lane] = s + pv[PV_CLS6_B + lane];
                    }
                } else {
                    float o = 0.f;
                    if (lane < 10) {
                        float s = 0.f;
                        for (int kh = 0; kh < un.b.KH; ++kh) s += P[(un.a.items + kh) * (R * 64) + row * 64 + lane];
                        const float r = s + pv[PV_REG4_B + lane];
                        const long long gi = live ? g : 0;
                        if (lane < 3) {
                            float p = a.bbox[gi * 10 + lane];
                            p = fminf(fmaxf(p, 0.f), 1.f);
                            const float logit = logf(fmaxf(p, 1e-5f) / fmaxf(1.f - p, 1e-5f));
                            o = 1.f / (1.f + expf(-(r + logit)));
                        } else {
                            o = r;
                            if (lane >= 8 && a.vel_div) o = r / a.vel_div[(unsigned)gi / (unsigned)a.Q];
                        }
                        if (live) a.box_out[g * 10 + lane] = o;
                    }
                    if (a.front) {
                        const int ob = (int)__float_as_uint(o);
                        const float x0 = __uint_as_float((unsigned)__builtin_amdgcn_readlane(ob, 0));
                        const float x1 = __uint_as_float((unsigned)__builtin_amdgcn_readlane(ob, 1));
                        const float x2 = __uint_as_float((unsigned)__builtin_amdgcn_readlane(ob, 2));
                        pe0_row<RG>(a, smem, row, lane, x0, x1, x2);
                    }
                }
            } break;
            case EPI_PE3: {
                if (side) break;
                if (PAIR && member == 0) {
                    pair_load4(px + (2 * R + row) * DM + lane * 4, v);
                    store_rows(smem, OFF_X2, LDX, row, lane, v);
                    break;
                }
                const LnW lw(pv + PV_PE4G, pv + PV_PE4B, lane);
                float res[4];
#pragma unroll
                for (int c = 0; c < 4; ++c) res[c] = smem[OFF_X3 + row * LDX + lane + 64 * c];
                gather4<R>(v, P, 0, un.a.KH, 0, row, lane, pv + PV_PE3_B, 0);
                ln4(v, lw, a.eps, true);
#pragma unroll
                for (int c = 0; c < 4; ++c) v[c] += res[c];
                store_rows(smem, OFF_X2, LDX, row, lane, v);
                if (PAIR) pair_store4(px + (2 * R + row) * DM + lane * 4, v);
                if (live) {
#pragma unroll
                    for (int c = 0; c < 4; ++c) a.x[g * DM + lane + 64 * c] = v[c];
                }
            } break;
            case EPI_QKV: {
                const int ncg = un.a.items / un.a.KH;
#pragma unroll
                for (int c = 0; c < 4; ++c) {
                    const int cg = side * 4 + c;
                    const int n = un.col0 + cg * 64 + lane;
                    if (cg < ncg && n < a.attn_in_rows) {
                        float s = 0.f;
                        for (int kh = 0; kh < un.a.KH; ++kh) s += P[(cg * un.a.KH + kh) * (R * 64) + row * 64 + lane];
                        if (live) a.qkvt[g * a.attn_in_rows + n] = s + pv[PV_QKV_B + n];
                    }
                }
            } break;
            case EPI_AOUT: {
                if (side) break;
                const LnW lw(pv + PV_N1G, pv + PV_N1B, lane);
                float res[4];
#pragma unroll
                for (int c = 0; c < 4; ++c) res[c] = smem[OFF_R + row * LDX + lane + 64 * c];
                gather4<R>(v, P, 0, un.a.KH, 0, row, lane, pv + PV_AOUT_B, 0);
#pragma unroll
                for (int c = 0; c < 4; ++c) v[c] += res[c];
                ln4(v, lw, a.eps, false);
                store_rows(smem, OFF_X3, LDX, row, lane, v);
                if (live) {
#pragma unroll
                    for (int c = 0; c < 4; ++c) a.x1_out[g * DM + lane + 64 * c] = v[c];
                }
                if (a.x1_frag && live) {
                    __builtin_amdgcn_wave_barrier();
                    const int k8 = lane & 31, im = lane >> 5;
                    const float up = a.x1_scale[0];
                    const float4 p0 = *reinterpret_cast<const float4*>(smem + OFF_X3 + row * LDX + 8 * k8);
                    const float4 p1 = *reinterpret_cast<const float4*>(smem + OFF_X3 + row * LDX + 8 * k8 + 4);
                    const float f[8] = {p0.x * up, p0.y * up, p0.z * up, p0.w * up, p1.x * up, p1.y * up, p1.z * up, p1.w * up};
                    unsigned w4[4];
#pragma unroll
                    for (int i = 0; i < 4; ++i) {
                        const _Float16 h0 = (_Float16)f[2 * i], h1 = (_Float16)f[2 * i + 1];
                        const _Float16 l0 = (_Float16)(f[2 * i] - (float)h0), l1 = (_Float16)(f[2 * i + 1] - (float)h1);
                        const _Float16 e0 = im ? l0 : h0, e1 = im ? l1 : h1;
                        w4[i] = (unsigned)__builtin_bit_cast(unsigned short, e0) | ((unsigned)__builtin_bit_cast(unsigned short, e1) << 16);
                    }
                    const long long frag = ((g >> 5) * (DM / 16) + (k8 >> 1)) * 2 + im;
                    uint4* dst = reinterpret_cast<uint4*>(a.x1_frag + frag * 512 + (((int)(g & 31) + 32 * (k8 & 1)) * 8));
                    *dst = make_uint4(w4[0], w4[1], w4[2], w4[3]);
                }
            } break;
            case EPI_SAMP: {
                if (side) break;
                const int ncg = un.a.items / un.a.KH;
#pragma unroll
                for (int c = 0; c < 4; ++c) {
                    const int n = c * 64 + lane;
                    if (c < ncg && n < a.soN) {
                        float s = 0.f;
                        for (int kh = 0; kh < un.a.KH; ++kh) s += P[(c * un.a.KH + kh) * (R * 64) + row * 64 + lane];
                        s += pv[PV_SAMP_B + n];
                        smem[OFF_H + row * 256 + n] = s;
                        if (live && a.so) a.so[g * a.soN + n] = s;
                    }
                }
            } break;
            }
        }
        SBEV_TRACE(4 + 4 * u)
        if (PAIR && un.epi == EPI_PE3 && member == 1) pair_arrive(pword);
        __syncthreads();
        SBEV_TRACE(5 + 4 * u)
    }
    if (PRE == PRE_ATT && a.proj.loc_bp) {
        const int GP = a.proj.G * a.proj.P;
        for (int i = threadIdx.x; i < R * a.proj.T * GP; i += 64 * NWAVE) {
            const int p = i % a.proj.P;
            const int row = (i / a.proj.P) % R;
            const int tg = i / (a.proj.P * R);
            const int gq = tg % a.proj.G, t = tg / a.proj.G;
            const long long g = row0 + row;
            if (g >= a.M) continue;
            const int b = (int)((unsigned)g / (unsigned)a.Q), q = (int)((unsigned)g - (unsigned)b * (unsigned)a.Q);
            const int gp = gq * a.proj.P + p;
            const float* so = smem + OFF_H + row * 256;
            sbev_ops::sample_point(a.proj, b, t, q, gp, a.proj.bbox + g * 10, so + gp * 3, so + GP * 3 + gp * a.proj.L);
        }
    }
}

__global__ void pack_kernel(const float* W, long long ld, int N, int K, float* out) {
    const long long i = (long long)blockIdx.x * 256 + threadIdx.x;
    const long long total = (long long)((N + 63) / 64) * K * 16;
    if (i >= total) return;
    const int lane = (int)(i & 63);
    const long long t = i >> 6;
    const int m = (int)(t & 3);
    const long long t2 = t >> 2;
    const int steps = K / 16;
    const int s = (int)(t2 % steps);
    const int cg = (int)(t2 / steps);
    const int n = cg * 64 + lane;
    float4 v = make_float4(0.f, 0.f, 0.f, 0.f);
    if (n < N) v = *reinterpret_cast<const float4*>(W + (long long)n * ld + 16 * s + 4 * m);
    reinterpret_cast<float4*>(out)[i] = v;
}

__global__ void copy_pad_kernel(const float* src, int n, float* dst, int slot) {
    const int i = blockIdx.x * 256 + threadIdx.x;
    if (i < slot) dst[i] = i < n ? src[i] : 0.f;
}

long long packed_floats(int N, int K) { return (long long)((N + 63) / 64) * 64 * K; }

struct PackMap {
    long long ffn0, ffn1, cls0, reg0, cls3, reg2, cls6, reg4, pe3, attn_in, attn_out, samp, vec, total;
};
PackMap pack_map(const sbev_decoder_config& c) {
    PackMap m{};
    long long o = 0;
    auto put = [&](long long& slot, int N, int K) { slot = o; o += packed_floats(N, K); };
    put(m.ffn0, c.ffn, c.D); put(m.ffn1, c.D, c.ffn);
    put(m.cls0, c.D, c.D); put(m.reg0, c.D, c.D); put(m.cls3, c.D, c.D); put(m.reg2, c.D, c.D);
    put(m.cls6, c.num_classes, c.D); put(m.reg4, c.code_size, c.D);
    put(m.pe3, c.D, c.D); put(m.attn_in, c.attn_in_rows, c.D);
    put(m.attn_out, c.D, c.D); put(m.samp, c.G * c.P * (3 + c.L), c.D);
    m.vec = o;
    m.total = o + PV_IMAGE_FLOATS;
    return m;
}

Lin lin(const float* wp, int in_off, int ld, int N, int K, int kh = 0, int cg0 = 0, int ncg = -1) {
    const int KH = kh > 0 ? kh : K / 128;
    const int all = (N + 63) / 64;
    if (ncg < 0) ncg = all - cg0;
    return Lin{wp + (long long)cg0 * K * 64, in_off, ld, KH, ncg * KH, K / (16 * KH), 0, KH};
}
Lin lin_khalf(const float* wp, int in_off, int ld, int N, int K, int kh, int half) {
    return Lin{wp, in_off, ld, kh, ((N + 63) / 64) * kh, K / (32 * kh), half * kh, 2 * kh};
}
const Lin kNone{nullptr, 0, LDX, 1, 0, 8, 0, 1};

int pieces(int rg, int cgs, int K) {
    if (rg == 1) return 0;
    static const bool tie_large = getenv("SBEV_CHAIN_TIE_SMALL") == nullptr;
    int best = 1;
    double best_cost = 1e30;
    for (int kh = 1; kh <= 4 && cgs * kh <= 12 && K / kh >= 16 * RDEPTH; kh *= 2) {
        const int items = cgs * kh, full = items / NWAVE, rest = items % NWAVE;
        const double cost = (K / (16.0 * kh)) * (full + (rest == 0 ? 0.0 : rest <= 4 ? 0.5 : 1.0));
        if (tie_large ? cost < best_cost + 1e-9 : cost < best_cost - 1e-9) { best_cost = cost; best = kh; }
    }
    return best;
}

int row_groups(long long rows) {
    static const int forced = getenv("SBEV_CHAIN_RG") ? atoi(getenv("SBEV_CHAIN_RG")) : 0;
    if ((forced == 1 && rows <= 256 * 4) || (forced == 2 && rows <= 256 * 8) || forced == 4) return forced;
    return rows <= 256 * 4 ? 1 : rows <= 256 * 8 ? 2 : 4;
}
Offs offs(int rg) { return rg == 1 ? offs_of<1>() : rg == 2 ? offs_of<2>() : offs_of<4>(); }

std::atomic<int> g_chain_pair{getenv("SBEV_NO_CHAIN_PAIR") ? 0 : 1};
std::atomic<int> g_chain_pair_drop{0};
std::atomic<unsigned> g_pair_fault_acked{0};
std::atomic<int> g_pair_fault_warned{0};
volatile unsigned* pair_fault_host() {
    static std::atomic<volatile unsigned*> word{nullptr};
    static std::mutex mu;
    volatile unsigned* w = word.load(std::memory_order_acquire);
    if (w) return w;
// ... 110 lines not shown
    const unsigned long long bit = 1ull << (dev & 63);
    if (done.load(std::memory_order_acquire) & bit) return hipSuccess;
    const hipError_t e = hipFuncSetAttribute(reinterpret_cast<const void*>(row_chain_kernel<PRE, RG, PAIR>),
                                             hipFuncAttributeMaxDynamicSharedMemorySize, Lay<RG>::LDS_TOTAL_FLOATS * 4);
    if (e == hipSuccess) done.fetch_or(bit, std::memory_order_release);
    return e;
}

template <int PRE, int RG, bool PAIR = false>
static int launch_t(const ChainArgs& a, hipStream_t s, const char* what) {
    constexpr int R = Lay<RG>::R, LDS_TOTAL_FLOATS = Lay<RG>::LDS_TOTAL_FLOATS;
    const hipError_t attr = lds_attr<PRE, RG, PAIR>();
    if (attr != hipSuccess) {
        set_error("%s: hipFuncSetAttribute(%d bytes of LDS): %s", what, LDS_TOTAL_FLOATS * 4, hipGetErrorString(attr));
        return SBEV_ELAUNCH;
    }
    static const bool no_warm = getenv("SBEV_CHAIN_NO_WARM") != nullptr;
    ChainArgs b = a;
    if (no_warm) b.warm_lines = 0;
#ifdef SBEV_CHAIN_TRACE
    static long long* tr = nullptr;
    static int calls = 0;
    if (!tr) { (void)hipMalloc(&tr, 2 * 64 * 8 * 8 * 64); (void)hipMemset(tr, 0, 2 * 64 * 8 * 8 * 64); }
    b.trace = tr + (calls % 64) * 512;
#endif
    const unsigned grid = PAIR ? (unsigned)pair_blocks(a.M, RG) : (unsigned)((a.M + R - 1) / R);
    hipLaunchKernelGGL((row_chain_kernel<PRE, RG, PAIR>), dim3(grid), dim3(64 * NWAVE), LDS_TOTAL_FLOATS * 4, s, b);
#ifdef SBEV_CHAIN_TRACE
    if (++calls == 13) {
        (void)hipDeviceSynchronize();
        static long long h[2 * 64 * 512];
        (void)hipMemcpy(h, tr, sizeof(h), hipMemcpyDeviceToHost);
        for (int c = 0; c < 13; ++c) {
            const long long* t = h + c * 512;
            printf("launch %d (PRE %d RG %d PAIR %d; 10 ns ticks):", c, PRE, RG, (int)PAIR);
            for (int blk = 0; blk < 2; ++blk)
                for (int w = 0; w < 8; w += 7) {
                    const long long* tb = t + blk * 64 * 512;
                    printf(" [b%d w%d]", blk ? 15 : 7, w);
                    for (int i = 0; i < 2 + 4 * 8 && tb[w * 64 + i]; ++i) printf(" %lld", tb[w * 64 + i] - t[0]);
                }
            printf("\n");
        }
    }
#endif
    return check_launch(what);
}

template <int RG>
static bool lds_ready_rg() {
    return lds_attr<PRE_SLABS, RG>() == hipSuccess && lds_attr<PRE_FRONT, RG>() == hipSuccess && lds_attr<PRE_ATT, RG>() == hipSuccess;
}
bool chain_lds_ready() {
    return lds_ready_rg<1>() && lds_ready_rg<2>() && lds_ready_rg<4>() && lds_attr<PRE_SLABS, 2, true>() == hipSuccess &&
           lds_attr<PRE_SLABS, 4, true>() == hipSuccess;
}

template <int RG>
static int launch_rg(const ChainArgs& a, hipStream_t s, const char* what) {
    return a.pre == PRE_SLABS ? launch_t<PRE_SLABS, RG>(a, s, what) : a.pre == PRE_FRONT ? launch_t<PRE_FRONT, RG>(a, s, what)
                                                                                          : launch_t<PRE_ATT, RG>(a, s, what);
}
static int launch(const ChainArgs& a, int rg, hipStream_t s, const char* what) {
    return rg == 1 ? launch_rg<1>(a, s, what) : rg == 2 ? launch_rg<2>(a, s, what) : launch_rg<4>(a, s, what);
}

int launch_chain_front(const sbev_decoder_config& c, const sbev_decoder_weights& w, const float* bbox, const float* feat, float* x,
                       float* qkvt, float eps, hipStream_t s, uint32_t* skip_hdr) {
    const PackMap m = pack_map(c);
    ChainArgs a{};
    fill_common(a, c, eps);
    a.pre = PRE_FRONT;
    a.bbox = bbox; a.feat = feat; a.x = x; a.qkvt = qkvt; a.skip_hdr = skip_hdr;
    const int rg = row_groups(a.M);
    a.n_units = add_front(a, 0, c, w.chain_pack, m, rg);
    a.warm = w.chain_pack + m.pe3;
    a.warm_lines = (int)((m.attn_out - m.pe3) / 32);
    a.vec = w.chain_pack + m.vec + PV_TAIL_END; a.vec_off = PV_TAIL_END; a.vec_n = PV_FRONT_END - PV_TAIL_END;
    return launch(a, rg, s, "row chain (front)");
}

int launch_chain_attn(const sbev_decoder_config& c, const sbev_decoder_weights& w, const float* att, const float* x, float* x1,
                      const float* bbox, const float* time_diff, const float* lidar2img, float* loc_bp, float* w_bp, float eps,
                      hipStream_t s, uint16_t* x1_frag, const float* x1_scale, uint32_t* pair_sync, const LazyPlan* touch, uint32_t* touch_need) {
    const PackMap m = pack_map(c);
    ChainArgs a{};
    fill_common(a, c, eps);
    a.pre = PRE_ATT;
    a.zero_words = pair_sync;
    a.n_zero = pair_sync ? (int)chain_pair_sync_words(a.M) : 0;
    a.att = att; a.x = const_cast<float*>(x); a.x1_out = x1; a.so = nullptr;
    a.x1_frag = x1_frag; a.x1_scale = x1_scale;
    a.proj = sbev_ops::sample_point_args(bbox, time_diff, lidar2img, c.pc_range, c.B, c.Q, c.T, c.N, c.G, c.P, c.L, c.image_h, c.image_w,
                                         c.eps_homo, loc_bp, w_bp);
    if (touch && touch_need) sbev_ops::sample_point_touch(a.proj, *touch, c.hw, touch_need);
    const int rg = row_groups(a.M);
    const Offs o = offs(rg);
    a.units[0] = Unit{lin(w.chain_pack + m.attn_out, o.x2, LDX, c.D, c.D, pieces(rg, c.D / 64, c.D)), kNone, EPI_AOUT, 0};
    a.units[1] = Unit{lin(w.chain_pack + m.samp, o.x3, LDX, a.soN, c.D, pieces(rg, (a.soN + 63) / 64, c.D)), kNone, EPI_SAMP, 0};
    a.n_units = 2;
    a.warm = w.chain_pack + m.attn_out;
    a.warm_lines = (int)((m.vec - m.attn_out) / 32);
    a.vec = w.chain_pack + m.vec + PV_FRONT_END; a.vec_off = 0; a.vec_n = PV_ATTN_END;
    return launch(a, rg, s, "row chain (attention)");
}

int launch_chain_tail(const sbev_decoder_config& c, const sbev_decoder_weights& w, const float* slabs, int splits, const float* x1,
                      const float* bbox, const float* vel_div, float* x3, float* cls_out, float* box_out, int with_front, float* x,
                      float* qkvt, float eps, hipStream_t s, float* pair_x, uint32_t* pair_sync) {
    const PackMap m = pack_map(c);
    const float* pk = w.chain_pack;
    ChainArgs a{};
    fill_common(a, c, eps);
    a.pre = PRE_SLABS;
    a.slabs = slabs; a.splits = splits; a.x1 = x1; a.bbox = bbox; a.vel_div = vel_div;
    a.x3 = x3; a.cls_out = cls_out; a.box_out = box_out; a.front = with_front; a.x = x; a.qkvt = qkvt;
    a.warm = pk + m.ffn0;
    a.warm_lines = (int)(((with_front ? m.attn_out : m.pe3) - m.ffn0) / 32);
    a.vec = pk + m.vec; a.vec_off = 0; a.vec_n = with_front ? PV_FRONT_END : PV_TAIL_END;
    const int dcg = c.D / 64;
    const int prg = pair_x && pair_sync ? pair_row_groups(a.M) : 0;
    if (prg) {
        const int rg = prg;
        const Offs o = offs(rg);
        const int half_cg = c.ffn / 128;
        const int kh1 = pieces(rg, dcg, c.ffn / 2);
        static const int q0_forced = getenv("SBEV_CHAIN_PAIR_Q0") ? atoi(getenv("SBEV_CHAIN_PAIR_Q0")) : -1;
        const int qcg = (c.attn_in_rows + 63) / 64;
        const int q0 = q0_forced >= 0 && q0_forced <= qcg ? q0_forced : (qcg > 8 ? qcg - 8 : qcg / 2);
        int n = 0;
        for (int mem = 0; mem < 2; ++mem) {
            Unit* u = mem ? a.units_b : a.units;
            n = 0;
            u[n++] = Unit{lin(pk + m.ffn0, o.x2, LDX, c.ffn, c.D, pieces(rg, half_cg, c.D), mem * half_cg, half_cg), kNone, EPI_FFN0, 0};
            u[n++] = Unit{lin_khalf(pk + m.ffn1, o.h, LDH, c.D, c.ffn, kh1, mem), kNone, EPI_FFN1, 0};
            const Lin br1 = lin(pk + (mem ? m.reg0 : m.cls0), o.x3, LDX, c.D, c.D, pieces(rg, dcg, c.D));
            const Lin br2 = lin(pk + (mem ? m.reg2 : m.cls3), mem ? o.r : o.c, LDX, c.D, c.D, pieces(rg, dcg, c.D));
            const Lin out = mem ? lin(pk + m.reg4, o.r, LDX, c.code_size, c.D, pieces(rg, 1, c.D)) : lin(pk + m.cls6, o.c, LDX, c.num_classes, c.D, pieces(rg, 1, c.D));
            u[n++] = mem ? Unit{kNone, br1, EPI_BR1, 0} : Unit{br1, kNone, EPI_BR1, 0};
            u[n++] = mem ? Unit{kNone, br2, EPI_BR2, 0} : Unit{br2, kNone, EPI_BR2, 0};
            u[n++] = mem ? Unit{kNone, out, EPI_OUT, 0} : Unit{out, kNone, EPI_OUT, 0};
            if (with_front) {
                u[n++] = Unit{mem ? lin(pk + m.pe3, o.c, LDX, c.D, c.D, pieces(rg, dcg, c.D)) : kNone, kNone, EPI_PE3, 0};
                const int cg0 = mem ? q0 : 0, ncg = mem ? qcg - q0 : q0;
                u[n++] = Unit{ncg > 0 ? lin(pk + m.attn_in, o.x2, LDX, c.attn_in_rows, c.D, pieces(rg, ncg, c.D), cg0, ncg) : kNone, kNone, EPI_QKV, cg0 * 64};
            }
        }
        a.n_units = n;
        a.n_pairs = (int)((a.M + 4 * rg - 1) / (4 * rg));
        a.pair_x = pair_x;
        a.pair_sync = pair_sync;
        a.debug_drop = g_chain_pair_drop.load(std::memory_order_relaxed);
        return rg == 2 ? launch_t<PRE_SLABS, 2, true>(a, s, "row chain (tail, pairs)") : launch_t<PRE_SLABS, 4, true>(a, s, "row chain (tail, pairs)");
    }
    int n = 0;
    const int rg = row_groups(a.M);
    const Offs o = offs(rg);
    a.units[n++] = Unit{lin(pk + m.ffn0, o.x2, LDX, c.ffn, c.D, pieces(rg, c.ffn / 64, c.D)), kNone, EPI_FFN0, 0};
    a.units[n++] = Unit{lin(pk + m.ffn1, o.h, LDH, c.D, c.ffn, pieces(rg, dcg, c.ffn)), kNone, EPI_FFN1, 0};
    a.units[n++] = Unit{lin(pk + m.cls0, o.x3, LDX, c.D, c.D, pieces(rg, 2 * dcg, c.D)), lin(pk + m.reg0, o.x3, LDX, c.D, c.D, pieces(rg, 2 * dcg, c.D)),
                        EPI_BR1, 0};
    a.units[n++] = Unit{lin(pk + m.cls3, o.c, LDX, c.D, c.D, pieces(rg, 2 * dcg, c.D)), lin(pk + m.reg2, o.r, LDX, c.D, c.D, pieces(rg, 2 * dcg, c.D)),
                        EPI_BR2, 0};
    a.units[n++] = Unit{lin(pk + m.cls6, o.c, LDX, c.num_classes, c.D, pieces(rg, 2, c.D)), lin(pk + m.reg4, o.r, LDX, c.code_size, c.D, pieces(rg, 2, c.D)),
                        EPI_OUT, 0};
    if (with_front) n = add_front(a, n, c, pk, m, rg);
    a.n_units = n;
    return launch(a, rg, s, "row chain (tail)");
}

}

extern "C" int sbev_decoder_chain_pair(int enable) { return g_chain_pair.exchange(enable != 0 ? 1 : 0); }

extern "C" int sbev_debug_chain_pair_drop(int enable) { return g_chain_pair_drop.exchange(enable != 0 ? 1 : 0); }

extern "C" int64_t sbev_decoder_chain_pair_timeouts(void) {
    unsigned v = 0;
    if (hipMemcpyFromSymbol(&v, HIP_SYMBOL(g_chain_pair_timeouts), sizeof(v)) != hipSuccess) return -1;
    const long long f = sbev::out_fold_timeouts();
    if (f < 0) return -1;
    return (int64_t)v + f;
}

extern "C" int64_t sbev_decoder_chain_pair_faults(void) { return (int64_t)sbev::chain_pair_faults_pending(); }
extern "C" int sbev_init(void) {
    if (g_chain_pair.load(std::memory_order_relaxed) == 0) return SBEV_OK;
    if (!pair_fault_install()) {
        sbev::set_error("sbev_init: could not install the pair-mode fault word on the current device (pair mode stays off until a later attempt succeeds)");
        return SBEV_ELAUNCH;
    }
    return SBEV_OK;
}
extern "C" int64_t sbev_decoder_chain_pair_faults_ack(void) {
    volatile unsigned* h = pair_fault_host();
    if (!h) return 0;
    const unsigned now = *h;
// ... 49 lines not shown
```

### sparsebev_amd/csrc/sbev_common.hpp

```cpp
#pragma once
#include <hip/hip_runtime.h>
#include <cstdarg>
#include <cstdint>
#include <cstdio>
#include <type_traits>

#include "../../include/sbev_hip.h"

namespace sbev {

void set_error(const char* fmt, ...);
int box_convention();

inline int check_launch(const char* what) {
    hipError_t e = hipGetLastError();
    if (e != hipSuccess) {
        set_error("%s: %s", what, hipGetErrorString(e));
        return SBEV_ELAUNCH;
    }
    return SBEV_OK;
}

#define SBEV_REQUIRE(cond, ...)                 \
    do {                                        \
// ... 64 lines not shown
    a.stride_g = d.stride_g; a.stride_px = d.stride_px;
    a.loc = d.loc; a.w = d.weights;
    a.N = d.N; a.C = d.C; a.Q = d.Q; a.P = d.P; a.gdiv = d.gdiv;
}
int msmv_fwd(const PyramidDesc& d, int64_t Bp, float* out, int out_layout, int T, int G, sbev_stream_t stream);
int sample_mix(const PyramidDesc& d, int64_t B, int T, int G, const float* params, float* y, int Pout, float eps, float out_up,
               const int32_t* order, sbev_stream_t stream);

struct SplitImageX {
    enum Form {
        F32_HOST_EXP,
        F16_PAIRS,
        F32_DEV_SCALE
    } form;
    const float* x;
    int64_t ldx;
    int up_log2;
    const float* dev_scale;
};
struct OutProj {
    SplitImageX X;
    const uint16_t* Wp;
    const float* nscale;
    int64_t M;
    int K, nimg;
    float* slabs;
    int out8_min_rows;
    unsigned* fold_sync;
    float* folded;
};
struct OutProjResult {
    int used;
    bool folded;
};
int launch_out_proj_slabs(const OutProj& o, OutProjResult* r, hipStream_t s);
bool out_fold_shape_ok(long long M, int K);
bool out_fold_enabled();
bool out_fold_install(void* host_word_dev);
long long out_fold_timeouts();
int out_fold_switch(int enable);
int out8_min_rows(int rows);
int out8_min_rows_setting();
int out_fold_drop(int enable);
bool gen_weight_stationary_enabled();

struct LazyPlan {
    int n_levels, R;
    long long n_images;
    int S[SBEV_MAX_LEVELS];
    unsigned tiles[SBEV_MAX_LEVELS];
    unsigned base[SBEV_MAX_LEVELS + 1];
};
bool lazy_plan(int n_levels, const int32_t* hw, long long n_images, int channels, LazyPlan* p);
struct LazyScan {
    const LazyPlan* plan;
    const void* const* table;
    const int32_t* index;
    const void* const* src;
    void* const* out;
    int esize;
    uint32_t *need, *done;
    bool last;
};
struct SplitFrags {
    const uint16_t* frags;
    const float* scale;
};
struct GenGemm {
    SplitFrags X, W;
    const float* bias;
    float* Y;
    int64_t M;
    int N, K;
    int64_t ldy;
    int relu, nimg;
    bool weight_stationary;
    const LazyScan* scan;
    const uint32_t* skip_hdr;
};
bool gen_ws_shape_ok(int64_t M, int K, int64_t ldy, int nimg);
int launch_gen_gemm(const GenGemm& g, hipStream_t s);
int launch_lazy_relayout(const LazyScan& scan, bool first, hipStream_t s);

bool row_chain_supported(const sbev_decoder_config& c);
bool row_chain_pays(long long rows);
int launch_chain_front(const sbev_decoder_config& c, const sbev_decoder_weights& w, const float* bbox, const float* feat, float* x,
                       float* qkvt, float eps, hipStream_t s, uint32_t* skip_hdr = nullptr);
int launch_sasa(const float* qkvt, int64_t ld, const float* query_bbox, const double* pc_range, const uint8_t* mask, float* out, int B, int Q,
                int H, int head_dim, const uint32_t* skip_hdr, hipStream_t s);
int launch_chain_attn(const sbev_decoder_config& c, const sbev_decoder_weights& w, const float* att, const float* x, float* x1,
                      const float* bbox, const float* time_diff, const float* lidar2img, float* loc_bp, float* w_bp, float eps,
                      hipStream_t s, uint16_t* x1_frag = nullptr, const float* x1_scale = nullptr, uint32_t* pair_sync = nullptr,
                      const LazyPlan* touch = nullptr, uint32_t* touch_need = nullptr);
int launch_sample_and_project(const float* query_bbox, const float* offset, int64_t ld_offset, const float* scale_logits, int64_t ld_logits,
                              const float* time_diff, const float* lidar2img, const double* pc_range, int B, int Q, int T, int N, int G, int P,
                              int L, float image_h, float image_w, float eps, float* loc_bp, float* weights_bp, const LazyPlan* touch,
                              uint32_t* touch_need, const int32_t (*hw)[2], hipStream_t stream);
int launch_chain_tail(const sbev_decoder_config& c, const sbev_decoder_weights& w, const float* slabs, int splits, const float* x1,
                      const float* bbox, const float* vel_div, float* x3, float* cls_out, float* box_out, int with_front, float* x,
                      float* qkvt, float eps, hipStream_t s, float* pair_x = nullptr, uint32_t* pair_sync = nullptr);
long long chain_pair_floats(long long rows);
long long chain_pair_sync_words(long long rows);
long long chain_fold_sync_offset(long long rows);
bool chain_pair_enabled();
bool chain_fault_word_ready();
void chain_pair_prepare();
unsigned chain_pair_faults_pending();

bool small_linear_shape(int64_t M, int N, int K);
int launch_ln_and_linear(const float* X, const float* ln_w, const float* ln_b, float eps, int ln_relu, float* Yln, int64_t M, int N,
                         const float* Xg, const float* W, const float* bias, float* Yg, int Ng, int K, int relu, hipStream_t s);
int launch_ln_and_refine(const float* X, const float* ln_w, const float* ln_b, float eps, int ln_relu, float* Yln, int64_t M, int N,
                         const float* bbox, const float* reg, const float* vel_div, float* out, int Q, int code, hipStream_t s);
int launch_linear_and_lin3(const float* Xg, const float* W, const float* bias, float* Yg, int64_t M, int Ng, int K, int relu,
                           const float* x3, int64_t ldx3, const float* w3, const float* b3, const float* ln_w, const float* ln_b,
                           float eps, float* y3, int N3, hipStream_t s);

struct LnPrologue {
    const float* g;
    const float* b;
    float eps;
    int relu;
    const float* add;
    float* xn;
};
int launch_linear_group(const sbev_linear_problem* probs, int n, const LnPrologue* ln, hipStream_t s);
bool ln_linear_fusable(int64_t M, int N, int K);

int launch_sasa_bwd_mfma(const float* qkvt, int64_t ld, const float* bbox, const float* lo, const float* span, const uint8_t* mask,
                         const float* out, const float* grad_out, float* grad_qkvt, float* lse, float* dvec,
                         int B, int Q, int H, float scale, float p_drop, uint64_t seed, const uint64_t* seed_dev, hipStream_t s);

bool profile_begin(hipStream_t s, hipEvent_t* e0, hipEvent_t* e1, int kind = 0);
void profile_end(hipStream_t s, hipEvent_t e0, hipEvent_t e1, int kind = 0);

constexpr int PFX_ARMED = 0, PFX_FORCE = 1, PFX_HITS = 2, PFX_MISSES = 3, PFX_DIRTY = 4, PFX_NW = 64;
__device__ __forceinline__ bool prefix_clean(const uint32_t* hdr) {
    const uint4* d = reinterpret_cast<const uint4*>(hdr + PFX_DIRTY);
    uint32_t acc = 0;
#pragma unroll
    for (int i = 0; i < PFX_NW / 4; ++i) {
        const uint4 v = d[i];
        acc |= (v.x | v.y) | (v.z | v.w);
    }
    return acc == 0;
}

__device__ __forceinline__ float wave_sum_dpp(float v) {
#define SBEV_DPP_F(x, ctrl) __uint_as_float((unsigned)__builtin_amdgcn_update_dpp(0, (int)__float_as_uint(x), ctrl, 0xf, 0xf, true))
    v += SBEV_DPP_F(v, 0x140);
    v += SBEV_DPP_F(v, 0x141);
    v += SBEV_DPP_F(v, 0x4e);
    v += SBEV_DPP_F(v, 0xb1);
#undef SBEV_DPP_F
    const int b = (int)__float_as_uint(v);
    const float r0 = __uint_as_float((unsigned)__builtin_amdgcn_readlane(b, 0));
    const float r1 = __uint_as_float((unsigned)__builtin_amdgcn_readlane(b, 16));
    const float r2 = __uint_as_float((unsigned)__builtin_amdgcn_readlane(b, 32));
    const float r3 = __uint_as_float((unsigned)__builtin_amdgcn_readlane(b, 48));
    return (r0 + r1) + (r2 + r3);
}

}
```

### sparsebev_amd/runtime.py

```python
import ctypes
import math
import os
import warnings
import weakref
from collections import namedtuple

import torch

from . import _lib
from .utils import frame_source

MAX_LEVELS = 5
GEMM_F32, GEMM_BF16X3, GEMM_BF16X6, GEMM_BF16X3S, GEMM_F16X3, GEMM_F16X4 = 0, 1, 2, 3, 4, 5
F16_MAX_HEADROOM_LOG2 = 12
GEMM_MODES = {'f32': GEMM_F32, 'bf16x3': GEMM_BF16X3, 'bf16x6': GEMM_BF16X6, 'bf16x3s': GEMM_BF16X3S, 'f16x3': GEMM_F16X3, 'f16x4': GEMM_F16X4}
_f = ctypes.c_void_p


class DecoderConfig(ctypes.Structure):
    _fields_ = [(n, ctypes.c_int32) for n in ('B', 'Q', 'T', 'N', 'G', 'P', 'L', 'D', 'H', 'ffn', 'num_classes',
                                              'code_size', 'num_layers', 'out_points', 'attn_in_rows', 'feat_dtype')] + \
               [('hw', (ctypes.c_int32 * 2) * MAX_LEVELS), ('image_h', ctypes.c_float), ('image_w', ctypes.c_float),
                ('eps_homo', ctypes.c_float), ('gemm_mode', ctypes.c_int32), ('n_slots', ctypes.c_int32),
                ('frame_slots', ctypes.c_int32 * 16), ('overlap', ctypes.c_int32),
                ('pc_range', ctypes.c_double * 6), ('slot_table', ctypes.c_void_p)]


_WEIGHT_FIELDS = ['pe0_w', 'pe0_b', 'pe1_g', 'pe1_b', 'pe3_w', 'pe3_b', 'pe4_g', 'pe4_b',
                  'attn_in_w', 'attn_in_b', 'attn_out_w', 'attn_out_b', 'samp_w', 'samp_b',
                  'pg_w', 'pg_b', 'op_w', 'op_b', 'pg_w2', 'op_w2', 'ffn0_w', 'ffn0_b', 'ffn1_w', 'ffn1_b',
                  'norm1_g', 'norm1_b', 'norm2_g', 'norm2_b', 'norm3_g', 'norm3_b',
                  'cls0_w', 'cls0_b', 'cls1_g', 'cls1_b', 'cls3_w', 'cls3_b', 'cls4_g', 'cls4_b', 'cls6_w', 'cls6_b',
                  'reg0_w', 'reg0_b', 'reg2_w', 'reg2_b', 'reg4_w', 'reg4_b', 'chain_pack', 'pg_ws', 'op_wp', 'pg_wdown', 'op_nscale', 'pg_xscale']


class DecoderWeights(ctypes.Structure):
    _fields_ = [(n, _f) for n in _WEIGHT_FIELDS]


class LazyFeats(ctypes.Structure):
    _fields_ = [('table', _f), ('index', ctypes.c_int32 * MAX_LEVELS), ('src', _f * MAX_LEVELS)]


def _ptr(t):
    return ctypes.c_void_p(t.data_ptr()) if t is not None else ctypes.c_void_p(0)


def _forward_cached(args, lazy, stream, prefix):
    lz = None
    if lazy is not None:
        lz = LazyFeats(table=lazy[1])
        (lz.src if lazy[1] is None else lz.index)[:len(lazy[0])] = lazy[0]
    pfx = (ctypes.c_void_p(prefix.ptr), prefix.nbytes) if prefix is not None else (None, 0)
    return _lib.load().sbev_decoder_forward_cached(*args[:_AFTER_FEATS], ctypes.byref(lz) if lz is not None else None, *args[_AFTER_FEATS:], stream, *pfx)


class PrefixCache:

    _live = None

    def __init__(self, nbytes, dev):
        self.nbytes, self.device = nbytes, dev
        self.buf = torch.empty(nbytes + 256, device=dev, dtype=torch.uint8)
        off = (-self.buf.data_ptr()) % 256
        self.ptr = self.buf.data_ptr() + off
        self.hdr = self.buf[off:off + 16].view(torch.int32)
        self.reset()
        if PrefixCache._live is None:
            PrefixCache._live = weakref.WeakSet()
        PrefixCache._live.add(self)

    def reset(self):
        self.hdr.zero_()
        self.force(_STATE['prefix_off'])

    def force(self, on):
        self.hdr[1:2].fill_(1 if on else 0)

    def counters(self):
        h = self.hdr.cpu()
        return int(h[2]), int(h[3])


def _prefix_cache_for(cfg, weights, mask, lazy, dev):
    lib = _lib.load()
    if _STATE['profile'] or lib.sbev_decoder_prefix_planned(ctypes.byref(cfg), ctypes.byref(weights), 1, int(mask is not None), int(bool(lazy))) != 1:
        return 0
    need = int(lib.sbev_prefix_cache_bytes(ctypes.byref(cfg)))
    limit = float(os.environ.get('SBEV_PREFIX_CACHE_MAX_MB', '1024')) * 2 ** 20
    return need if 0 < need <= limit else 0


class DecoderRuntime:

    def __init__(self, decoder, gemm_mode=0, overlap=False):
        if os.environ.get('SBEV_NO_SAMPLE_MIX') == '1':
            fuse_sample_mix(False)
        if os.environ.get('SBEV_NO_ROW_CHAIN') == '1':
            row_chain(False)
        self.decoder = decoder
        self.gemm_mode = gemm_mode
        self.overlap = overlap
        self._sig = None
        self._keep = None
        self._weights = None
        self._ws = None
        self._ws_key = None
        self._params = None
        self._graph_ws = {}
        self._sig_calls = 0
        self.mode_eff = gemm_mode
        self.f16_headroom_log2 = 0.0
        self.step_graphs = StepGraphs(self)
        self._prefix = None
        self._prefix_key = None

    def _signature(self):
        self._sig_calls += 1
        if self._params is None or (self._sig_calls & 63) == 0:
            self._params = [(m._parameters, n) for m in self.decoder.modules() for n, p in m._parameters.items() if p is not None]
        try:
            ps = [d[n] for d, n in self._params]
            return tuple((p.data_ptr(), p._version) for p in ps)
        except (KeyError, AttributeError):
            self._params = [(m._parameters, n) for m in self.decoder.modules() for n, p in m._parameters.items() if p is not None]
            return tuple((d[n].data_ptr(), d[n]._version) for d, n in self._params)

    def _ensure_bound(self):
        sig = self._signature()
        if sig != self._sig:
            rebind = self._sig is not None
            self._bind()
            self._sig = sig
            if rebind:
                self.step_graphs.clear()
        return sig

# ... 353 lines not shown
                    None if table is None else (table.data_ptr(), tuple(table.shape)), ins), [], False
        if all(self._relayout_ok(f) for f in feats):
            return ('nchw', tuple((tuple(f.shape), f.dtype) for f in feats)), [], True
        return ('list', tuple((f.data_ptr(), tuple(f.shape), tuple(f.stride()), f.dtype) for f in feats)), list(feats), False

    def run(self, query_bbox, query_feat, mlvl_feats, attn_mask, img_metas, finish=False, src=None):
        rt = self.rt
        if _STATE['profile'] or not (query_bbox.is_cuda and query_bbox.is_contiguous() and query_feat.is_contiguous()):
            return None
        if query_bbox.data_ptr() % 16 or query_feat.data_ptr() % 16:
            return None
        if attn_mask is not None and not (attn_mask.is_cuda and attn_mask.dtype == torch.uint8 and attn_mask.is_contiguous() and attn_mask.data_ptr() % 16 == 0):
            return None
        src = src or frame_source(mlvl_feats)
        if src.kind == 'list' and not all(torch.is_tensor(f) and f.is_cuda for f in mlvl_feats):
            return None
        from . import transformer as TR
        check_pair_faults()
        sig = rt._ensure_bound()
        fkey, ident, staged = self._feat_key(mlvl_feats, src)
        key = StepKey(tuple(query_bbox.shape), tuple(query_feat.shape), fkey, None if attn_mask is None else tuple(attn_mask.shape), sig,
                      torch.cuda.current_device(), _switch_key(), rt.decoder.num_layers, tuple(rt.decoder.pc_range),
                      torch.cuda.current_stream(query_bbox.device).cuda_stream, bool(finish))
        verdict, e = self.admit(key, ident, pinned=not staged and not src.resident)
        if e is None:
            return None
        B, Q = query_bbox.shape[:2]
        packed, layout, ih, iw = consts = TR.DecoderContext.pack(img_metas, B)
        outs = None
        if finish:
            nl, nc, cs = rt.decoder.num_layers, rt.decoder.decoder_layer.num_classes, rt.decoder.decoder_layer.code_size
            outs = (torch.empty(nl, B, Q, nc, device=query_bbox.device, dtype=torch.float32),
                    torch.empty(nl, B, Q, cs, device=query_bbox.device, dtype=torch.float32))
        call = StepInputs(query_bbox, query_feat, mlvl_feats, attn_mask, outs, None if src.insert is None else src.insert.frames)
        if verdict == CAPTURE:
            e = self._capture(key, call, consts, staged, src)
            if e is None:
                return None
        else:
            if layout != e.layout or (ih, iw) != e.image:
                return None
            TR._upload(self._with_table(packed, e.n_packed, e.staged, call), query_bbox.device, out=e.ctx_buf)
        self.launch(key, e)
        return outs if outs is not None else (e.graph.cls, e.graph.box)

    @staticmethod
    def _with_table(packed, n_packed, staged, call):
        import numpy as np
        ptrs = [call.bbox.data_ptr(), call.feat.data_ptr(), call.mask.data_ptr() if call.mask is not None else 0]
        if staged:
            ptrs += [f.data_ptr() for f in call.feats]
        elif call.frames is not None:
            ptrs += [f.data_ptr() for f in call.frames]
        if call.outs is not None:
            ptrs += [call.outs[0].data_ptr(), call.outs[1].data_ptr()]
        full = np.empty(n_packed + 2 * len(ptrs), dtype=np.float32)
        full[:packed.size] = packed
        full[packed.size:n_packed] = 0.0
        full[n_packed:].view(np.int64)[:] = ptrs
        return full

    def _capture(self, key, call, consts, staged, src):
        from . import transformer as TR
        rt, dev = self.rt, call.bbox.device
        packed, layout, ih, iw = consts
        qb, qf = torch.empty_like(call.bbox), torch.empty_like(call.feat)
        mask = torch.empty_like(call.mask) if call.mask is not None else None
        pyramid = TR.FeaturePyramid.for_graph(call.feats, staged) if src.kind == 'list' else call.feats
        if pyramid is None:
            return None
        insert = None
        if src.insert is not None:
            pyramid = pyramid.resident()
            insert = (list(range(3, 3 + len(call.frames))), src.insert, pyramid)
        n_packed = (packed.size + 3) // 4 * 4
        ctx = TR.DecoderContext.from_packed(self._with_table(packed, n_packed, staged, call), layout, ih, iw, dev)
        args, keep, cls, box = rt._prepare(qb, qf, pyramid, ctx, mask, own_workspace=True)
        try:
            segs = [(0, qb), (1, qf)] + ([(2, mask)] if mask is not None else [])
            relayout = [(3 + l, buf) for l, buf in enumerate(pyramid.levels)] if staged else []
            lazy = len(relayout) > 0 and _STATE['lazy'] and bool(_lib.load().sbev_decoder_lazy_supported(args.config))
            need = _prefix_cache_for(keep.cfg, rt._weights, mask, lazy, dev)
            prefix = PrefixCache(need, dev) if need else None
            handle = self._record(args, ctypes.c_void_p(ctx.buffer.data_ptr() + 4 * n_packed), segs, relayout, lazy,
                                  (cls, box) if call.outs is not None else None, insert, prefix)
        except BaseException:
            rt._release_graph_ws(keep.ws_key)
            raise
        graph = DecoderGraph(handle, (keep, qb, qf, mask, ctx, None if staged else (None if insert else call.feats, pyramid)), cls, box)
        e = CapturedStep(graph, not staged and not src.resident, staged, ctx.buffer, n_packed, layout, (ih, iw), keep.ws_key, prefix)
        self.captured(key, e)
        return e

    @staticmethod
    def _record(args, table, segs, relayout, lazy, finish, insert=None, prefix=None):
        lib = _lib.load()
        side = torch.cuda.Stream(device=segs[0][1].device)
        side.wait_stream(torch.cuda.current_stream())
        sp = ctypes.c_void_p(side.cuda_stream)
        c_idx = (ctypes.c_int32 * len(segs))(*[i for i, _ in segs])
        c_dst = (ctypes.c_void_p * len(segs))(*[t.data_ptr() for _, t in segs])
        c_nb = (ctypes.c_int64 * len(segs))(*[t.numel() * t.element_size() for _, t in segs])
        n = len(relayout)
        n_img, ch = relayout[0][1].shape[::3] if n else (0, 0)
        hws = [buf.shape[1] * buf.shape[2] for _, buf in relayout]
        _lib.check(lib.sbev_capture_begin(sp), 'sbev_capture_begin')
        ok, st_fwd = True, 0
        try:
            ok = lib.sbev_copy_indirect(table, len(segs), c_idx, c_dst, c_nb, sp) == 0
            multi = (not lazy and 1 < n <= MAX_LEVELS and ch % 4 == 0 and _STATE['relayout_multi']
                     and all(buf.dtype == torch.float32 and hw % 4 == 0 for (_, buf), hw in zip(relayout, hws)))
            if multi:
                c_ix = (ctypes.c_int32 * n)(*[i for i, _ in relayout])
                c_out = (ctypes.c_void_p * n)(*[buf.data_ptr() for _, buf in relayout])
                ok = ok and lib.sbev_nchw_to_nhwc_f32_multi_indirect(table, n, c_ix, c_out, n_img, ch, (ctypes.c_int32 * n)(*hws), sp) == 0
            elif not lazy:
                for (idx, buf), hw in zip(relayout, hws):
                    fn = lib.sbev_nchw_to_nhwc_f32_indirect if buf.dtype == torch.float32 else lib.sbev_nchw_to_nhwc_b16_indirect
                    ok = ok and fn(table, idx, _ptr(buf), n_img, ch, hw, sp) == 0
            if insert is not None and ok:
                from . import cache
                idx, pending, pool_pyr = insert
                ok = cache.pool_insert_frames(pending.frames, pool_pyr.levels, pending.rows, pool_pyr.n_slots, sp, pending.nhwc, table, idx, check=False) == 0
            st_fwd = _forward_cached(args, ([idx for idx, _ in relayout], table) if lazy else None, sp, prefix) if ok else 0
            ok = ok and st_fwd == 0
            if finish is not None:
                cls, box = finish
                i_out = 3 + (n if insert is None else len(insert[0]))
                ok = ok and lib.sbev_finish_outputs_indirect(table, i_out, i_out + 1, _ptr(cls), _ptr(box), cls.numel(), box.numel(), sp) == 0
        finally:
            handle = ctypes.c_void_p()
            st = lib.sbev_capture_end(sp, ctypes.byref(handle) if ok else None)
        if st_fwd == _lib.EFAULT:
            _lib.check(st_fwd, 'sbev_decoder_forward (capture)')
        if not ok:
            raise _lib.SbevError('graph capture of the decoder step failed: ' + lib.sbev_last_error().decode())
        _lib.check(st, 'sbev_capture_end')
        torch.cuda.current_stream().wait_stream(side)
        return handle


class _FirstSighting:

    def __init__(self, tensors):
        self.refs = [(weakref.ref(t.untyped_storage()), t.storage_offset(), tuple(t.shape), tuple(t.stride()), t.dtype) for t in tensors]

    def same(self, tensors):
        return len(tensors) == len(self.refs) and all(
            r[0]() is not None and r[0]() is t.untyped_storage() and r[1:] == (t.storage_offset(), tuple(t.shape), tuple(t.stride()), t.dtype)
            for r, t in zip(self.refs, tensors))


class DecoderGraph:

    def __init__(self, handle, keep, cls, box):
        self._h, self._keep, self.cls, self.box = handle, keep, cls, box
        self.num_nodes = int(_lib.load().sbev_graph_num_nodes(handle))

    def replay(self):
        if self._h is None:
            raise RuntimeError('DecoderGraph was destroyed')
        st = _lib.load().sbev_graph_launch(self._h, ctypes.c_void_p(torch.cuda.current_stream().cuda_stream))
        _lib.check(st, 'sbev_graph_launch')
        return self.cls, self.box

    def destroy(self):
        if self._h is not None:
            _lib.load().sbev_graph_destroy(self._h)
            self._h = None

    def __del__(self):
        try:
            self.destroy()
        except Exception:
            pass


class _State(dict):
    def __missing__(self, key):
        if key != 'order':
            raise KeyError(key)
        return _switch_key()[4]


_STATE = _State(profile=0,
                prefix_off=os.environ.get('SBEV_NO_PREFIX_CACHE') == '1',
                lazy=not os.environ.get('SBEV_NO_SPARSE_RELAYOUT'),
                relayout_multi=not os.environ.get('SBEV_NO_RELAYOUT_MULTI'))


def _switch_key():
    buf = (ctypes.c_int32 * 32)()
    n = _lib.load().sbev_decoder_switches(buf, 32)
    assert 0 < n <= 32
    return tuple(buf[:n]) + (bool(_STATE['lazy']), bool(_STATE['relayout_multi']))


def out_fold(enable):
    return bool(_lib.load().sbev_decoder_out_fold(int(bool(enable))))


def prefix_cache(enable):
    prev = not _STATE['prefix_off']
    _STATE['prefix_off'] = not enable
    for c in list(PrefixCache._live or ()):
        with torch.cuda.device(c.device):
            c.force(not enable)
    return prev


def lazy_relayout(enable):
# ... 64 lines not shown
```

Measured before the change: 580.6 samples/s.

## Fold query staging into prefix watch and output finishing into chain tails

The captured decoder step used to start with an indirect copy of the query bbox and feature into staging buffers and end with a separate indirect finish-outputs launch. The prefix-watch kernel now reads the queries through the pointer table, stages them and compares them in one pass, and the row-chain tail kernels write cls/box straight to the caller's output pointers. The aim is to drop two graph nodes and the extra memory passes they make. The prefix cache also keeps x1 and the sampling-offset result instead of x0/att0, which changes what layer 0 can skip. The watch loop is unrolled four ways, and the change adds new API surface and indexing assumptions tied to the pointer-table layout.

```diff
diff --git a/include/sbev_hip.h b/include/sbev_hip.h
--- a/include/sbev_hip.h
+++ b/include/sbev_hip.h
@@ -478,6 +478,19 @@
                                 void* workspace, int64_t workspace_bytes, sbev_stream_t stream, void* cache, int64_t cache_bytes);
 int sbev_decoder_prefix_planned(const sbev_decoder_config* cfg, const sbev_decoder_weights* weights, int cache_given, int mask_given,
                                 int lazy_given);
+typedef struct sbev_step_edges {
+    const void* const* table;
+    int32_t idx_bbox, idx_feat;
+    int32_t idx_cls, idx_box;
+} sbev_step_edges;
+int sbev_decoder_edges_planned(const sbev_decoder_config* cfg, const sbev_decoder_weights* weights, int cache_given, int mask_given,
+                               int lazy_given);
+int sbev_decoder_forward_edges(const sbev_decoder_config* cfg, const sbev_decoder_weights* weights, void* const* feats_nhwc,
+                               const sbev_lazy_feats* lazy, float* query_bbox, float* query_feat,
+                               const float* time_diff, const float* lidar2img, const float* vel_div,
+                               const uint8_t* attn_mask, float* cls_out, float* bbox_out,
+                               void* workspace, int64_t workspace_bytes, sbev_stream_t stream, void* cache, int64_t cache_bytes,
+                               const sbev_step_edges* edges);
 int64_t sbev_lazy_relayout_tiles(int n_levels, const int32_t* hw_pixels, int64_t n_images, int channels);
 int sbev_sample_and_project_touch(const float* query_bbox, const float* offset, int64_t ld_offset,
                                   const float* scale_logits, int64_t ld_logits,
diff --git a/sparsebev_amd/_lib.py b/sparsebev_amd/_lib.py
--- a/sparsebev_amd/_lib.py
+++ b/sparsebev_amd/_lib.py
@@ -63,6 +63,9 @@
                                                    _vp, ctypes.c_int64, _vp, _vp, ctypes.c_int64]),
     'sbev_prefix_cache_bytes': (ctypes.c_int64, [_vp]),
     'sbev_decoder_prefix_planned': (ctypes.c_int, [_vp, _vp, ctypes.c_int, ctypes.c_int, ctypes.c_int]),
+    'sbev_decoder_edges_planned': (ctypes.c_int, [_vp, _vp, ctypes.c_int, ctypes.c_int, ctypes.c_int]),
+    'sbev_decoder_forward_edges': (ctypes.c_int, [_vp, _vp, ctypes.POINTER(_vp), _vp, _vp, _vp, _vp, _vp, _vp, _vp, _vp, _vp,
+                                                  _vp, ctypes.c_int64, _vp, _vp, ctypes.c_int64, _vp]),
     'sbev_decoder_lazy_supported': (ctypes.c_int, [_vp]),
     'sbev_decoder_lazy_scan_launch': (ctypes.c_int, [ctypes.c_int]),
     'sbev_lazy_relayout_tiles': (ctypes.c_int64, [ctypes.c_int, _c_i32p, ctypes.c_int64, ctypes.c_int]),
diff --git a/sparsebev_amd/csrc/decoder.hip b/sparsebev_amd/csrc/decoder.hip
--- a/sparsebev_amd/csrc/decoder.hip
+++ b/sparsebev_amd/csrc/decoder.hip
@@ -82,7 +82,7 @@
 
 struct Prefix {
     uint32_t* hdr;
-    float *qb, *qf, *x0, *att0, *params0;
+    float *qb, *qf, *x1_0, *so_0, *params0;
     size_t bytes;
 };
 Prefix carve_prefix(const sbev_decoder_config& c, void* cache) {
@@ -93,8 +93,8 @@
     f.hdr = reinterpret_cast<uint32_t*>(k.take(sbev::PFX_DIRTY + sbev::PFX_NW));
     f.qb = k.take(BQ * 10);
     f.qf = k.take(BQ * D);
-    f.x0 = k.take(BQ * D);
-    f.att0 = k.take(BQ * D);
+    f.x1_0 = k.take(BQ * D);
+    f.so_0 = k.take(BQ * D);
     f.params0 = k.take(BQ * (size_t)c.G * (Cg * Cg + Pin * c.out_points));
     f.bytes = k.off;
     return f;
@@ -105,26 +105,49 @@
     uint32_t* copy[2];
     uint32_t words[2];
     uint32_t* hdr;
+    const void* const* table;
+    int idx[2];
+    uint32_t* stage[2];
 };
 __global__ __launch_bounds__(256) void prefix_watch_kernel(const WatchArgs a) {
     const uint32_t armed = a.hdr[sbev::PFX_ARMED], force = a.hdr[sbev::PFX_FORCE];
     uint32_t differed = 0;
 #pragma unroll
     for (int s = 0; s < 2; ++s) {
-        const uint4* q = reinterpret_cast<const uint4*>(a.q[s]);
+        const uint32_t* qw = a.table ? static_cast<const uint32_t*>(a.table[a.idx[s]]) : a.q[s];
+        uint32_t* const sw = a.table ? a.stage[s] : nullptr;
+        const uint4* q = reinterpret_cast<const uint4*>(qw);
         uint4* cp = reinterpret_cast<uint4*>(a.copy[s]);
+        uint4* st = reinterpret_cast<uint4*>(sw);
         const uint32_t n16 = a.words[s] / 4;
-        for (uint32_t i = blockIdx.x * 256u + threadIdx.x; i < n16; i += sbev::PFX_NW * 256u) {
-            const uint4 v = q[i], o = cp[i];
-            if (((v.x ^ o.x) | (v.y ^ o.y)) | ((v.z ^ o.z) | (v.w ^ o.w))) {
-                cp[i] = v;
-                differed = 1;
+        constexpr uint32_t PASS = sbev::PFX_NW * 256u;
+        for (uint32_t i0 = blockIdx.x * 256u + threadIdx.x; i0 < n16; i0 += 4u * PASS) {
+            uint4 v[4], o[4];
+#pragma unroll
+            for (uint32_t k = 0; k < 4u; ++k) {
+                const uint32_t i = i0 + k * PASS, j = i < n16 ? i : i0;
+                v[k] = q[j];
+                o[k] = cp[j];
+            }
+#pragma unroll
+            for (uint32_t k = 0; k < 4u; ++k) {
+                const uint32_t i = i0 + k * PASS;
+                if (i >= n16) continue;
+                if (st) st[i] = v[k];
+                if (((v[k].x ^ o[k].x) | (v[k].y ^ o[k].y)) | ((v[k].z ^ o[k].z) | (v[k].w ^ o[k].w))) {
+                    cp[i] = v[k];
+                    differed = 1;
+                }
             }
         }
         const uint32_t t = 4 * n16 + threadIdx.x;
-        if (blockIdx.x == 0 && t < a.words[s] && a.q[s][t] != a.copy[s][t]) {
-            a.copy[s][t] = a.q[s][t];
-            differed = 1;
+        if (blockIdx.x == 0 && t < a.words[s]) {
+            const uint32_t v = qw[t];
+            if (sw) sw[t] = v;
+            if (v != a.copy[s][t]) {
+                a.copy[s][t] = v;
+                differed = 1;
+            }
         }
     }
     const int any = __syncthreads_or((int)differed);
@@ -313,6 +336,13 @@
     return plan_step(*cfg, *w, lazy_given != 0, true, read_switches(), cache_given && !mask_given && !launch_profiling_on()).prefix ? 1 : 0;
 }
 
+extern "C" int sbev_decoder_edges_planned(const sbev_decoder_config* cfg, const sbev_decoder_weights* w, int cache_given, int mask_given,
+                                          int lazy_given) {
+    if (validate(cfg) != SBEV_OK || !w) return -1;
+    const StepPlan p = plan_step(*cfg, *w, lazy_given != 0, true, read_switches(), cache_given && !mask_given && !launch_profiling_on());
+    return (p.prefix ? 1 : 0) | (p.chain ? 2 : 0);
+}
+
 extern "C" int64_t sbev_decoder_workspace_bytes(const sbev_decoder_config* cfg) {
     if (validate(cfg) != SBEV_OK) return -1;
     sbev::chain_pair_prepare();
@@ -332,6 +362,7 @@
     float *cls_out, *bbox_out;
     const sbev_lazy_feats* lazy;
     const Prefix* pf;
+    const sbev_step_edges* ed;
     sbev_stream_t stream;
     Aux& ax;
     hipStream_t s_main = reinterpret_cast<hipStream_t>(stream);
@@ -346,6 +377,7 @@
     bool pe0_done = false;
     hipEvent_t ev_cls = nullptr;
     float* params = b.params;
+    float* x1 = b.x1;
     const uint32_t* skip = nullptr;
 
     float* cls_of(int layer) const { return cls_out + (int64_t)layer * p.BQ * c.num_classes; }
@@ -370,16 +402,16 @@
     int lazy_move(const sbev::LazyScan& scan, bool first) { return scan.plan ? sbev::launch_lazy_relayout(scan, first, s_main) : SBEV_OK; }
 
     int generator_bf16x3(sbev_stream_t st) {
-        if (!p.pg_strip) return sbev_linear_bf16x3(b.x1, w.pg_w2, w.pg_b, nullptr, params, p.BQ, p.pgN, D, D, p.pgN, 0, st);
+        if (!p.pg_strip) return sbev_linear_bf16x3(x1, w.pg_w2, w.pg_b, nullptr, params, p.BQ, p.pgN, D, D, p.pgN, 0, st);
         uint16_t* x2 = reinterpret_cast<uint16_t*>(b.x1s);
-        TRY(sbev_split_bf16x3_weights(b.x1, x2, p.BQ, D, st));
+        TRY(sbev_split_bf16x3_weights(x1, x2, p.BQ, D, st));
         return sbev_linear_bf16x3_strip(x2, w.pg_w2, w.pg_b, params, p.BQ, p.pgN, D, p.pgN, 0, st);
     }
     int generator_bf16s(sbev_stream_t st, const sbev::LazyScan* scan) {
         uint16_t* xs = reinterpret_cast<uint16_t*>(b.x1s);
         if (p.pack_launch) {
-            TRY(p.nimg >= 4 ? sbev_pack_f16s_frags(b.x1, D, xs, const_cast<float*>(w.pg_xscale), (int)p.BQ, D, 2, st)
-                            : sbev_pack_bf16s_frags(b.x1, D, xs, (int)p.BQ, D, p.nimg, st));
+            TRY(p.nimg >= 4 ? sbev_pack_f16s_frags(x1, D, xs, const_cast<float*>(w.pg_xscale), (int)p.BQ, D, 2, st)
+                            : sbev_pack_bf16s_frags(x1, D, xs, (int)p.BQ, D, p.nimg, st));
         }
         return sbev::launch_gen_gemm({{xs, w.pg_xscale}, {w.pg_ws, w.pg_wdown}, w.pg_b, params, p.BQ, p.pgN, D, p.pgN, 0, p.nimg, p.gen_ws, scan, skip},
                                      reinterpret_cast<hipStream_t>(st));
@@ -387,7 +419,7 @@
     int generator(sbev_stream_t st, const sbev::LazyScan* scan) {
         if (p.nimg) return generator_bf16s(st, scan);
         if (c.gemm_mode == SBEV_GEMM_BF16X3) return generator_bf16x3(st);
-        return sbev_linear_f32(b.x1, w.pg_w, w.pg_b, nullptr, params, p.BQ, p.pgN, D, D, D, p.pgN, 0, st);
+        return sbev_linear_f32(x1, w.pg_w, w.pg_b, nullptr, params, p.BQ, p.pgN, D, D, D, p.pgN, 0, st);
     }
 
     int gather(sbev_stream_t st) {
@@ -432,13 +464,13 @@
     int layer_chain(int layer) {
         if (p.order_mode != 0 && (layer == 0 || p.order_mode == 1)) TRY(sbev_query_order(bbox, c.code_size, c.pc_range, c.B, c.Q, b.order, stream));
         const bool cached = pf && layer == 0;
-        float* att = cached ? pf->att0 : b.att;
+        x1 = cached ? pf->x1_0 : b.x1;
         params = cached ? pf->params0 : b.params;
         skip = cached ? pf->hdr : nullptr;
-        TRY(sbev::launch_sasa(b.qkvt, c.attn_in_rows, bbox, c.pc_range, attn_mask, att, c.B, c.Q, c.H, D / c.H, skip, s_main));
-        TRY(sbev::launch_chain_attn(c, w, att, cached ? pf->x0 : b.x, b.x1, bbox, time_diff, lidar2img, b.loc, b.wbp, eps, s_main,
+        TRY(sbev::launch_sasa(b.qkvt, c.attn_in_rows, bbox, c.pc_range, attn_mask, b.att, c.B, c.Q, c.H, D / c.H, skip, s_main));
+        TRY(sbev::launch_chain_attn(c, w, b.att, b.x, x1, bbox, time_diff, lidar2img, b.loc, b.wbp, eps, s_main,
                                     p.nimg >= 4 ? reinterpret_cast<uint16_t*>(b.x1s) : nullptr, p.nimg >= 4 ? w.pg_xscale : nullptr, b.pair_sync,
-                                    lazy ? &lplan : nullptr, lazy ? b.touch_need : nullptr));
+                                    lazy ? &lplan : nullptr, lazy ? b.touch_need : nullptr, skip, cached ? pf->so_0 : nullptr));
         const bool ride = p.scan_in_gen && layer > 0;
         SBEV_REQUIRE(!(ride && skip), "sbev_decoder_forward: a generator that carries a relayout scan cannot skip");
         const sbev::LazyScan scan = lazy_scan(layer);
@@ -447,8 +479,11 @@
         TRY(gather_and_mix(stream, p.order_mode != 0 ? b.order : nullptr));
         sbev::OutProjResult op;
         TRY(out_projection_slabs(&op));
-        TRY(sbev::launch_chain_tail(c, w, op.folded ? b.folded : b.slabs, op.used, b.x1, bbox, c.T > 1 ? vel_div : nullptr, b.x3, cls_of(layer), box_of(layer),
-                                    layer + 1 < c.num_layers, b.x, b.qkvt, eps, s_main, b.pair_x, b.pair_sync));
+        const bool finish = ed && ed->idx_cls >= 0;
+        const sbev::ChainFinish fin{finish ? ed->table : nullptr, finish ? ed->idx_cls : 0, finish ? ed->idx_box : 0,
+                                    (long long)layer * p.BQ * c.num_classes, (long long)layer * p.BQ * c.code_size};
+        TRY(sbev::launch_chain_tail(c, w, op.folded ? b.folded : b.slabs, op.used, x1, bbox, c.T > 1 ? vel_div : nullptr, b.x3, cls_of(layer), box_of(layer),
+                                    layer + 1 < c.num_layers, b.x, b.qkvt, eps, s_main, b.pair_x, b.pair_sync, finish ? &fin : nullptr));
         bbox = box_of(layer);
         return SBEV_OK;
     }
@@ -520,16 +555,20 @@
     }
 
     int prefix_watch() {
+        const bool stage = ed && ed->idx_bbox >= 0;
         const WatchArgs a{{reinterpret_cast<const uint32_t*>(query_bbox), reinterpret_cast<const uint32_t*>(query_feat)},
                           {reinterpret_cast<uint32_t*>(pf->qb), reinterpret_cast<uint32_t*>(pf->qf)},
-                          {(uint32_t)(p.BQ * 10), (uint32_t)(p.BQ * D)}, pf->hdr};
+                          {(uint32_t)(p.BQ * 10), (uint32_t)(p.BQ * D)}, pf->hdr,
+                          stage ? ed->table : nullptr, {stage ? ed->idx_bbox : 0, stage ? ed->idx_feat : 0},
+                          {stage ? reinterpret_cast<uint32_t*>(const_cast<float*>(query_bbox)) : nullptr,
+                           stage ? reinterpret_cast<uint32_t*>(const_cast<float*>(query_feat)) : nullptr}};
         hipLaunchKernelGGL(prefix_watch_kernel, dim3(sbev::PFX_NW), dim3(256), 0, s_main, a);
         return sbev::check_launch("prefix cache (watch)");
     }
 
     int run() {
         if (pf) TRY(prefix_watch());
-        if (p.chain) TRY(sbev::launch_chain_front(c, w, query_bbox, query_feat, pf ? pf->x0 : b.x, b.qkvt, eps, s_main, pf ? pf->hdr : nullptr));
+        if (p.chain) TRY(sbev::launch_chain_front(c, w, query_bbox, query_feat, b.x, b.qkvt, eps, s_main, pf ? pf->hdr : nullptr));
         for (int layer = 0; layer < c.num_layers; ++layer) TRY(p.chain ? layer_chain(layer) : layer_ops(layer));
         return join(ev_cls);
     }
@@ -542,7 +581,7 @@
                                 const float* time_diff, const float* lidar2img, const float* vel_div,
                                 const uint8_t* attn_mask, float* cls_out, float* bbox_out,
                                 void* workspace, int64_t workspace_bytes, sbev_stream_t stream, const sbev_lazy_feats* lazy,
-                                void* cache = nullptr, int64_t cache_bytes = 0) {
+                                void* cache = nullptr, int64_t cache_bytes = 0, const sbev_step_edges* edges = nullptr) {
     TRY(validate(cfg));
     const sbev_decoder_config& c = *cfg;
     SBEV_REQUIRE(w && feats_nhwc && query_bbox && query_feat && time_diff && lidar2img && cls_out && bbox_out && workspace,
@@ -571,8 +610,18 @@
         SBEV_REQUIRE((int64_t)pf.bytes <= cache_bytes, "sbev_decoder_forward_cached: cache too small (%lld < %zu)", (long long)cache_bytes, pf.bytes);
         SBEV_REQUIRE(p.BQ * (int64_t)c.D < 0x7fffffffLL, "sbev_decoder_forward_cached: too many query words");
     }
+    if (edges) {
+        const bool stage = edges->idx_bbox >= 0 || edges->idx_feat >= 0, finish = edges->idx_cls >= 0 || edges->idx_box >= 0;
+        SBEV_REQUIRE(!(stage || finish) || (edges->table && (((uintptr_t)edges->table) & 7) == 0), "sbev_decoder_forward_edges: null / unaligned pointer table");
+        SBEV_REQUIRE(!stage || (edges->idx_bbox >= 0 && edges->idx_feat >= 0), "sbev_decoder_forward_edges: idx_bbox and idx_feat come together");
+        SBEV_REQUIRE(!finish || (edges->idx_cls >= 0 && edges->idx_box >= 0), "sbev_decoder_forward_edges: idx_cls and idx_box come together");
+        SBEV_REQUIRE(!stage || p.prefix, "sbev_decoder_forward_edges: the queries are staged by the prefix cache's watch launch, which this step does not have "
+                                         "(sbev_decoder_edges_planned)");
+        SBEV_REQUIRE(!finish || p.chain, "sbev_decoder_forward_edges: the outputs are finished by the row-chain tails, which this step does not run "
+                                         "(sbev_decoder_edges_planned)");
+    }
     Step step{c, *w, p, b, feats_nhwc, query_bbox, query_feat, time_diff, lidar2img, vel_div, attn_mask, cls_out, bbox_out, lazy,
-              p.prefix ? &pf : nullptr, stream, ax};
+              p.prefix ? &pf : nullptr, edges, stream, ax};
     if (lazy) {
         SBEV_REQUIRE(lazy_plan_of(c, &step.lplan) && b.touch_need, "sbev_decoder_forward_lazy: config not covered (dense pyramid, 4 groups of 64 channels)");
         for (int l = 0; l < c.L; ++l)
@@ -613,6 +662,16 @@
                                            void* workspace, int64_t workspace_bytes, sbev_stream_t stream, void* cache, int64_t cache_bytes) {
     return decoder_forward_impl(cfg, w, const_cast<const void* const*>(feats_nhwc), query_bbox, query_feat, time_diff, lidar2img, vel_div, attn_mask,
                                 cls_out, bbox_out, workspace, workspace_bytes, stream, lazy, cache, cache_bytes);
+}
+
+extern "C" int sbev_decoder_forward_edges(const sbev_decoder_config* cfg, const sbev_decoder_weights* w, void* const* feats_nhwc,
+                                          const sbev_lazy_feats* lazy, float* query_bbox, float* query_feat,
+                                          const float* time_diff, const float* lidar2img, const float* vel_div,
+                                          const uint8_t* attn_mask, float* cls_out, float* bbox_out,
+                                          void* workspace, int64_t workspace_bytes, sbev_stream_t stream, void* cache, int64_t cache_bytes,
+                                          const sbev_step_edges* edges) {
+    return decoder_forward_impl(cfg, w, const_cast<const void* const*>(feats_nhwc), query_bbox, query_feat, time_diff, lidar2img, vel_div, attn_mask,
+                                cls_out, bbox_out, workspace, workspace_bytes, stream, lazy, cache, cache_bytes, edges);
 }
 
 extern "C" int sbev_decoder_lazy_supported(const sbev_decoder_config* cfg) {
diff --git a/sparsebev_amd/csrc/row_chain.hip b/sparsebev_amd/csrc/row_chain.hip
--- a/sparsebev_amd/csrc/row_chain.hip
+++ b/sparsebev_amd/csrc/row_chain.hip
@@ -78,10 +78,20 @@
     unsigned short* x1_frag;
     const float* x1_scale;
     float* so; int soN;
-    sbev_ops::SamplePointArgs proj;
+    union {
+        sbev_ops::SamplePointArgs proj;
+        struct { const void* const* table; int idx_cls, idx_box; long long off_cls, off_box; } fin;
+    };
     float eps;
     uint32_t* skip_hdr;
 };
+
+__device__ __forceinline__ float finish1(float v) {
+    const unsigned u = __float_as_uint(v), e = u & 0x7f800000u;
+    if (e != 0x7f800000u) return v;
+    if (u & 0x007fffffu) return 0.f;
+    return __uint_as_float((u & 0x80000000u) | 0x7f7fffffu);
+}
 
 constexpr int RING_SLOTS = 3;
 constexpr int CHUNK_FLOATS = 1024;
@@ -394,6 +404,24 @@
     store_rows(smem, OFF_C, LDX, row, lane, v);
 }
 
+template <int RG>
+__device__ __forceinline__ void place_points(const ChainArgs& a, const float* smem, long long row0) {
+    constexpr int R = Lay<RG>::R, OFF_H = Lay<RG>::OFF_H;
+    const int GP = a.proj.G * a.proj.P;
+    for (int i = threadIdx.x; i < R * a.proj.T * GP; i += 64 * NWAVE) {
+        const int p = i % a.proj.P;
+        const int row = (i / a.proj.P) % R;
+        const int tg = i / (a.proj.P * R);
+        const int gq = tg % a.proj.G, t = tg / a.proj.G;
+        const long long g = row0 + row;
+        if (g >= a.M) continue;
+        const int b = (int)((unsigned)g / (unsigned)a.Q), q = (int)((unsigned)g - (unsigned)b * (unsigned)a.Q);
+        const int gp = gq * a.proj.P + p;
+        const float* so = smem + OFF_H + row * 256;
+        sbev_ops::sample_point(a.proj, b, t, q, gp, a.proj.bbox + g * 10, so + gp * 3, so + GP * 3 + gp * a.proj.L);
+    }
+}
+
 template <int PRE, int RG, bool PAIR = false>
 __global__ __launch_bounds__(64 * NWAVE) void row_chain_kernel(const ChainArgs a) {
     using L = Lay<RG>;
@@ -416,6 +444,13 @@
     float* const px = PAIR ? a.pair_x + (long long)pair * (3 * R * DM) : nullptr;
     const long long row0 = (long long)pair * R;
     float* P = smem + OFF_P;
+    float *fin_cls = nullptr, *fin_box = nullptr;
+    if constexpr (PRE == PRE_SLABS) {
+        if (a.fin.table) {
+            fin_cls = static_cast<float*>(const_cast<void*>(a.fin.table[a.fin.idx_cls])) + a.fin.off_cls;
+            fin_box = static_cast<float*>(const_cast<void*>(a.fin.table[a.fin.idx_box])) + a.fin.off_box;
+        }
+    }
     if constexpr (PRE == PRE_FRONT) {
         if (a.skip_hdr) {
             const bool clean = sbev::prefix_clean(a.skip_hdr);
@@ -428,6 +463,18 @@
     }
     if (PRE == PRE_ATT && a.zero_words && blockIdx.x == 0)
         for (int i = threadIdx.x; i < a.n_zero; i += 64 * NWAVE) a.zero_words[i] = 0u;
+    if constexpr (PRE == PRE_ATT) {
+        if (a.skip_hdr && sbev::prefix_clean(a.skip_hdr)) {
+            for (int i = threadIdx.x; i < R * a.soN; i += 64 * NWAVE) {
+                const int row = i / a.soN, n = i - row * a.soN;
+                const long long g = row0 + row;
+                if (g < a.M) smem[OFF_H + row * 256 + n] = a.so[g * a.soN + n];
+            }
+            __syncthreads();
+            if (a.proj.loc_bp) place_points<RG>(a, smem, row0);
+            return;
+        }
+    }
 
     SBEV_TRACE(0)
     warm_l2<RG>(a, wave, lane);
@@ -626,6 +673,9 @@
                         float s = 0.f;
                         for (int kh = 0; kh < un.a.KH; ++kh) s += P[kh * (R * 64) + row * 64 + lane];
                         if (live) a.cls_out[g * a.num_classes + lane] = s + pv[PV_CLS6_B + lane];
+                        if constexpr (PRE == PRE_SLABS) {
+                            if (live && fin_cls) fin_cls[g * a.num_classes + lane] = finish1(s + pv[PV_CLS6_B + lane]);
+                        }
                     }
                 } else {
                     float o = 0.f;
@@ -644,6 +694,9 @@
                             if (lane >= 8 && a.vel_div) o = r / a.vel_div[(unsigned)gi / (unsigned)a.Q];
                         }
                         if (live) a.box_out[g * 10 + lane] = o;
+                        if constexpr (PRE == PRE_SLABS) {
+                            if (live && fin_box) fin_box[g * 10 + lane] = finish1(o);
+                        }
                     }
                     if (a.front) {
                         const int ob = (int)__float_as_uint(o);
@@ -746,21 +799,7 @@
         __syncthreads();
         SBEV_TRACE(5 + 4 * u)
     }
-    if (PRE == PRE_ATT && a.proj.loc_bp) {
-        const int GP = a.proj.G * a.proj.P;
-        for (int i = threadIdx.x; i < R * a.proj.T * GP; i += 64 * NWAVE) {
-            const int p = i % a.proj.P;
-            const int row = (i / a.proj.P) % R;
-            const int tg = i / (a.proj.P * R);
-            const int gq = tg % a.proj.G, t = tg / a.proj.G;
-            const long long g = row0 + row;
-            if (g >= a.M) continue;
-            const int b = (int)((unsigned)g / (unsigned)a.Q), q = (int)((unsigned)g - (unsigned)b * (unsigned)a.Q);
-            const int gp = gq * a.proj.P + p;
-            const float* so = smem + OFF_H + row * 256;
-            sbev_ops::sample_point(a.proj, b, t, q, gp, a.proj.bbox + g * 10, so + gp * 3, so + GP * 3 + gp * a.proj.L);
-        }
-    }
+    if (PRE == PRE_ATT && a.proj.loc_bp) place_points<RG>(a, smem, row0);
 }
 
 __global__ void pack_kernel(const float* W, long long ld, int N, int K, float* out) {
@@ -1037,14 +1076,20 @@
 
 int launch_chain_attn(const sbev_decoder_config& c, const sbev_decoder_weights& w, const float* att, const float* x, float* x1,
                       const float* bbox, const float* time_diff, const float* lidar2img, float* loc_bp, float* w_bp, float eps,
-                      hipStream_t s, uint16_t* x1_frag, const float* x1_scale, uint32_t* pair_sync, const LazyPlan* touch, uint32_t* touch_need) {
+                      hipStream_t s, uint16_t* x1_frag, const float* x1_scale, uint32_t* pair_sync, const LazyPlan* touch, uint32_t* touch_need,
+                      const uint32_t* skip_hdr, float* so_keep) {
     const PackMap m = pack_map(c);
     ChainArgs a{};
     fill_common(a, c, eps);
     a.pre = PRE_ATT;
+    if ((skip_hdr != nullptr) != (so_keep != nullptr) || (skip_hdr && (!loc_bp || !x1))) {
+        set_error("row chain (attention): a prefix cache header comes with the cached so rows, x1 rows and the in-kernel projection");
+        return SBEV_EINVAL;
+    }
+    a.skip_hdr = const_cast<uint32_t*>(skip_hdr);
     a.zero_words = pair_sync;
     a.n_zero = pair_sync ? (int)chain_pair_sync_words(a.M) : 0;
-    a.att = att; a.x = const_cast<float*>(x); a.x1_out = x1; a.so = nullptr;
+    a.att = att; a.x = const_cast<float*>(x); a.x1_out = x1; a.so = so_keep;
     a.x1_frag = x1_frag; a.x1_scale = x1_scale;
     a.proj = sbev_ops::sample_point_args(bbox, time_diff, lidar2img, c.pc_range, c.B, c.Q, c.T, c.N, c.G, c.P, c.L, c.image_h, c.image_w,
                                          c.eps_homo, loc_bp, w_bp);
@@ -1062,12 +1107,20 @@
 
 int launch_chain_tail(const sbev_decoder_config& c, const sbev_decoder_weights& w, const float* slabs, int splits, const float* x1,
                       const float* bbox, const float* vel_div, float* x3, float* cls_out, float* box_out, int with_front, float* x,
-                      float* qkvt, float eps, hipStream_t s, float* pair_x, uint32_t* pair_sync) {
+                      float* qkvt, float eps, hipStream_t s, float* pair_x, uint32_t* pair_sync, const ChainFinish* fin) {
     const PackMap m = pack_map(c);
     const float* pk = w.chain_pack;
     ChainArgs a{};
     fill_common(a, c, eps);
     a.pre = PRE_SLABS;
+    if (fin) {
+        if (!fin->table || (((uintptr_t)fin->table) & 7) != 0 || fin->idx_cls < 0 || fin->idx_box < 0 || fin->off_cls < 0 || fin->off_box < 0) {
+            set_error("row chain (tail): finished outputs need an 8-byte aligned pointer table and indices / offsets >= 0");
+            return SBEV_EINVAL;
+        }
+        a.fin.table = fin->table; a.fin.idx_cls = fin->idx_cls; a.fin.idx_box = fin->idx_box;
+        a.fin.off_cls = fin->off_cls; a.fin.off_box = fin->off_box;
+    }
     a.slabs = slabs; a.splits = splits; a.x1 = x1; a.bbox = bbox; a.vel_div = vel_div;
     a.x3 = x3; a.cls_out = cls_out; a.box_out = box_out; a.front = with_front; a.x = x; a.qkvt = qkvt;
     a.warm = pk + m.ffn0;
diff --git a/sparsebev_amd/csrc/sbev_common.hpp b/sparsebev_amd/csrc/sbev_common.hpp
--- a/sparsebev_amd/csrc/sbev_common.hpp
+++ b/sparsebev_amd/csrc/sbev_common.hpp
@@ -170,6 +170,11 @@
 int launch_gen_gemm(const GenGemm& g, hipStream_t s);
 int launch_lazy_relayout(const LazyScan& scan, bool first, hipStream_t s);
 
+struct ChainFinish {
+    const void* const* table;
+    int idx_cls, idx_box;
+    long long off_cls, off_box;
+};
 bool row_chain_supported(const sbev_decoder_config& c);
 bool row_chain_pays(long long rows);
 int launch_chain_front(const sbev_decoder_config& c, const sbev_decoder_weights& w, const float* bbox, const float* feat, float* x,
@@ -179,14 +184,15 @@
 int launch_chain_attn(const sbev_decoder_config& c, const sbev_decoder_weights& w, const float* att, const float* x, float* x1,
                       const float* bbox, const float* time_diff, const float* lidar2img, float* loc_bp, float* w_bp, float eps,
                       hipStream_t s, uint16_t* x1_frag = nullptr, const float* x1_scale = nullptr, uint32_t* pair_sync = nullptr,
-                      const LazyPlan* touch = nullptr, uint32_t* touch_need = nullptr);
+                      const LazyPlan* touch = nullptr, uint32_t* touch_need = nullptr, const uint32_t* skip_hdr = nullptr, float* so_keep = nullptr);
 int launch_sample_and_project(const float* query_bbox, const float* offset, int64_t ld_offset, const float* scale_logits, int64_t ld_logits,
                               const float* time_diff, const float* lidar2img, const double* pc_range, int B, int Q, int T, int N, int G, int P,
                               int L, float image_h, float image_w, float eps, float* loc_bp, float* weights_bp, const LazyPlan* touch,
                               uint32_t* touch_need, const int32_t (*hw)[2], hipStream_t stream);
 int launch_chain_tail(const sbev_decoder_config& c, const sbev_decoder_weights& w, const float* slabs, int splits, const float* x1,
                       const float* bbox, const float* vel_div, float* x3, float* cls_out, float* box_out, int with_front, float* x,
-                      float* qkvt, float eps, hipStream_t s, float* pair_x = nullptr, uint32_t* pair_sync = nullptr);
+                      float* qkvt, float eps, hipStream_t s, float* pair_x = nullptr, uint32_t* pair_sync = nullptr,
+                      const ChainFinish* fin = nullptr);
 long long chain_pair_floats(long long rows);
 long long chain_pair_sync_words(long long rows);
 long long chain_fold_sync_offset(long long rows);
diff --git a/sparsebev_amd/runtime.py b/sparsebev_amd/runtime.py
--- a/sparsebev_amd/runtime.py
+++ b/sparsebev_amd/runtime.py
@@ -46,13 +46,19 @@
     return ctypes.c_void_p(t.data_ptr()) if t is not None else ctypes.c_void_p(0)
 
 
-def _forward_cached(args, lazy, stream, prefix):
+class StepEdges(ctypes.Structure):
+    _fields_ = [('table', _f), ('idx_bbox', ctypes.c_int32), ('idx_feat', ctypes.c_int32), ('idx_cls', ctypes.c_int32), ('idx_box', ctypes.c_int32)]
+
+
+def _forward_cached(args, lazy, stream, prefix, edges=None):
     lz = None
     if lazy is not None:
         lz = LazyFeats(table=lazy[1])
         (lz.src if lazy[1] is None else lz.index)[:len(lazy[0])] = lazy[0]
     pfx = (ctypes.c_void_p(prefix.ptr), prefix.nbytes) if prefix is not None else (None, 0)
-    return _lib.load().sbev_decoder_forward_cached(*args[:_AFTER_FEATS], ctypes.byref(lz) if lz is not None else None, *args[_AFTER_FEATS:], stream, *pfx)
+    lib = _lib.load()
+    head = (*args[:_AFTER_FEATS], ctypes.byref(lz) if lz is not None else None, *args[_AFTER_FEATS:], stream, *pfx)
+    return lib.sbev_decoder_forward_cached(*head) if edges is None else lib.sbev_decoder_forward_edges(*head, ctypes.byref(edges))
 
 
 class PrefixCache:
@@ -572,8 +578,10 @@
             lazy = len(relayout) > 0 and _STATE['lazy'] and bool(_lib.load().sbev_decoder_lazy_supported(args.config))
             need = _prefix_cache_for(keep.cfg, rt._weights, mask, lazy, dev)
             prefix = PrefixCache(need, dev) if need else None
+            inside = _lib.load().sbev_decoder_edges_planned(ctypes.byref(keep.cfg), ctypes.byref(rt._weights), int(prefix is not None),
+                                                            int(mask is not None), int(bool(lazy)))
             handle = self._record(args, ctypes.c_void_p(ctx.buffer.data_ptr() + 4 * n_packed), segs, relayout, lazy,
-                                  (cls, box) if call.outs is not None else None, insert, prefix)
+                                  (cls, box) if call.outs is not None else None, insert, prefix, max(inside, 0))
         except BaseException:
             rt._release_graph_ws(keep.ws_key)
             raise
@@ -583,9 +591,15 @@
         return e
 
     @staticmethod
-    def _record(args, table, segs, relayout, lazy, finish, insert=None, prefix=None):
+    def _record(args, table, segs, relayout, lazy, finish, insert=None, prefix=None, inside=0):
         lib = _lib.load()
-        side = torch.cuda.Stream(device=segs[0][1].device)
+        i_out = 3 + (len(relayout) if insert is None else len(insert[0]))
+        edges = StepEdges(table=table, idx_bbox=0 if inside & 1 else -1, idx_feat=1 if inside & 1 else -1,
+                          idx_cls=i_out if inside & 2 and finish is not None else -1, idx_box=i_out + 1 if inside & 2 and finish is not None else -1)
+        dev = segs[0][1].device
+        if inside & 1:
+            segs = [sg for sg in segs if sg[0] > 1]
+        side = torch.cuda.Stream(device=dev)
         side.wait_stream(torch.cuda.current_stream())
         sp = ctypes.c_void_p(side.cuda_stream)
         c_idx = (ctypes.c_int32 * len(segs))(*[i for i, _ in segs])
@@ -597,7 +611,7 @@
         _lib.check(lib.sbev_capture_begin(sp), 'sbev_capture_begin')
         ok, st_fwd = True, 0
         try:
-            ok = lib.sbev_copy_indirect(table, len(segs), c_idx, c_dst, c_nb, sp) == 0
+            ok = not segs or lib.sbev_copy_indirect(table, len(segs), c_idx, c_dst, c_nb, sp) == 0
             multi = (not lazy and 1 < n <= MAX_LEVELS and ch % 4 == 0 and _STATE['relayout_multi']
                      and all(buf.dtype == torch.float32 and hw % 4 == 0 for (_, buf), hw in zip(relayout, hws)))
             if multi:
@@ -612,11 +626,11 @@
                 from . import cache
                 idx, pending, pool_pyr = insert
                 ok = cache.pool_insert_frames(pending.frames, pool_pyr.levels, pending.rows, pool_pyr.n_slots, sp, pending.nhwc, table, idx, check=False) == 0
-            st_fwd = _forward_cached(args, ([idx for idx, _ in relayout], table) if lazy else None, sp, prefix) if ok else 0
+            st_fwd = _forward_cached(args, ([idx for idx, _ in relayout], table) if lazy else None, sp, prefix,
+                                     edges if inside & 3 else None) if ok else 0
             ok = ok and st_fwd == 0
-            if finish is not None:
+            if finish is not None and edges.idx_cls < 0:
                 cls, box = finish
-                i_out = 3 + (n if insert is None else len(insert[0]))
                 ok = ok and lib.sbev_finish_outputs_indirect(table, i_out, i_out + 1, _ptr(cls), _ptr(box), cls.numel(), box.numel(), sp) == 0
         finally:
             handle = ctypes.c_void_p()
```

Result: no change. 580.5 samples/s (-0.0%).
